# proycon/colibri-core

Measured on AMD Instinct MI355X. Metric: M patterns counted/sec at n<=5 thr=2; identical pattern set vs reference, higher is better.
Workload: dtype u64; 1 GPU; 100000000-token-per-GPU synthetic Zipf(1.0, V=1000000) class-encoded corpus (.colibri.dat v2), sentences 5..35 tokens, unindexed PatternModel<uint32_t>, MAXLENGTH=5, MINTOKENS=2; patterns_in_model=9386566, parallelism=single device

## Files before the change

### colibri-core_amd/csrc/bigram2.hpp

```cpp
#pragma once
#ifndef COLIBRI_BI2_HUGE
#define COLIBRI_BI2_HUGE 16384
#endif
#include "bi2_mix.hpp"
#include "binned.hpp"

namespace colibri {

#ifndef COLIBRI_BI2_CNT16
#define COLIBRI_BI2_CNT16 1
#endif
#ifndef COLIBRI_BI2_WEU
#define COLIBRI_BI2_WEU 4
#endif
constexpr int bi2_count_weu(int slots, bool key4, bool based) { return (COLIBRI_BI2_CNT16 && slots == 1024 && !key4 && !based) ? 5 : COLIBRI_BI2_WEU; }
#ifndef COLIBRI_BI2_WROWS
#define COLIBRI_BI2_WROWS 12
#endif
#ifndef COLIBRI_BI2_WSLOTS
#define COLIBRI_BI2_WSLOTS 1024
#endif
#ifndef COLIBRI_BI2_BINTARGET
#define COLIBRI_BI2_BINTARGET 700
#endif
// ... 1232 lines not shown
        const uint32_t excl = bi2_block_scan<kBi2BigThreads>(nk, &ktotal, wsumL);
        bi2_block_scan<kBi2BigThreads>(nu, &distinct, wsumL);
        if (distinct > kMaxLoad || ktotal > 1023u) {
            if (tid == 0) bs->overflow = 2;
            continue;
        }
        if (tid == 0) {
            atomicAdd(&bs->found_part[a], distinct);
            bs->binkept[a * kBi2BBins + b] = ktotal;
            if (ktotal) atomicAdd(&bs->kept_part[a], ktotal);
        }
        if (ktotal == 0) {
            if (KEY4)
                for (uint32_t j = tid; j < total; j += kBi2BigThreads) code_at[locate(j)] = kInvalid;
            continue;
        }
        const bool reps_lds = ktotal <= (uint32_t)kBi2WReps;
        {
            uint32_t r = excl;
#pragma unroll
            for (uint32_t i = 0; i < per; ++i) {
                if (cS[i] >= threshold) {
                    sp_cnt[spo + r] = cS[i];
                    cntT[s0 + i]    = kBi2Kept | r;
                    if (reps_lds)
                        repS[r] = 0xFFFFFFFFu;
                    else
                        sp_rep[spo + r] = 0xFFFFFFFFu;
                    ++r;
                }
            }
        }
        if (!reps_lds) __threadfence();
        __syncthreads();
        const uint32_t fcode = (a * (uint32_t)kBi2BBins + b) << 10;
        for (uint32_t j0 = 0; j0 < total; j0 += kBi2BigRows * kBi2BigThreads) {
            load4(j0);
#pragma unroll
            for (int q = 0; q < kBi2BigRows; ++q) {
                if (j0 + q * kBi2BigThreads + (tid & ~(uint32_t)(kWave - 1)) >= total) continue;
                const bool     valid = y[q] != ~0ull;
                const uint32_t key = (uint32_t)(y[q] >> pb) & 0x7FFFFFFFu;
                uint32_t       pos = (uint32_t)(y[q] & pmask);
                if (PDROP && pdsh != 0u) {
                    uint32_t jj = j0 + q * kBi2BigThreads + tid, sub = 0;
#pragma unroll
                    for (int s2 = 0; s2 < NSUB - 1; ++s2) {
                        const bool beyond = jj >= rn[s2] && sub == (uint32_t)s2;
                        jj -= beyond ? rn[s2] : 0u;
                        sub += beyond ? 1u : 0u;
                    }
                    const uint32_t sh = pdsh - 1u;
                    pos               = ((pos >> sh) << (sh + 3u)) | (sub << sh) | (pos & ((1u << sh) - 1u));
                }
                uint32_t       c = 0;
                if (valid) c = cntT[bi2_find(keyT, key, bi2_bucket_of(key, lgb, bmask), bmask)];
                const bool     kept = (c & kBi2Kept) != 0;
                const uint32_t r    = c & ~kBi2Kept;
                if (KEY4 && valid) code_at[pos] = kept ? (fcode | r) : kInvalid;
                if (kept) {
                    if (reps_lds) {
                        if (pos < repS[r]) atomicMin(&repS[r], pos);
                    } else if (pos < __hip_atomic_load(&sp_rep[spo + r], __ATOMIC_RELAXED, __HIP_MEMORY_SCOPE_AGENT)) {
                        atomicMin(&sp_rep[spo + r], pos);
                    }
                }
                if (want_positions && !KEY4) {
                    const uint64_t m = __ballot(kept);
                    const uint32_t n = (uint32_t)__popcll(m);
                    if (n && (chunk == kInvalid || cursor + n > csize)) {
                        if (chunk != kInvalid && lane == 0) wcnt[chunk] = cursor;
                        uint32_t cc = 0;
                        if (lane == 0) cc = atomicAdd(&bs->nextchunk, 1u);
                        cc     = (uint32_t)__builtin_amdgcn_readfirstlane((int)cc);
                        chunk  = cc < pn ? pfirst + cc : kInvalid;
                        cursor = 0;
                        if (chunk == kInvalid) lost = true;
                    }
                    if (kept && chunk != kInvalid) {
                        const size_t at = (size_t)chunk * csize + cursor + (uint32_t)__popcll(m & ((1ull << lane) - 1ull));
                        wlist[at]       = pos;
                        if (wcode != nullptr) wcode[at] = fcode | r;
                    }
                    if (chunk != kInvalid) cursor += n;
                }
            }
        }
        __syncthreads();
        if (reps_lds)
            for (uint32_t r = tid; r < ktotal; r += kBi2BigThreads) sp_rep[spo + r] = repS[r];
    }
    if (want_positions && chunk != kInvalid && lane == 0) wcnt[chunk] = cursor;
    if (__any(lost) && lane == 0) bs->overflow = 3;
}

__global__ void bi2_chunk_cursor_kernel(Bi2State* __restrict__ bs, uint32_t* __restrict__ keep, bool restore) {
    if (restore)
        bs->nextchunk = *keep;
    else
        *keep = bs->nextchunk;
}
__global__ __launch_bounds__(kBi2BBins) void bi2_kept_scan_kernel(Bi2State* __restrict__ bs, const DevState* __restrict__ st) {
    if (st->done) return;
    __shared__ uint32_t inL[kBi2BBins], outL[kBi2BBins], wsumL[8], beforeL;
    const uint32_t      a = blockIdx.x;
    inL[threadIdx.x]      = threadIdx.x < a ? bs->kept_part[threadIdx.x] : 0u;
    __syncthreads();
    const uint32_t before = bi2_scan512(inL, outL, wsumL);
    if (threadIdx.x == 0) beforeL = before;
    __syncthreads();
    inL[threadIdx.x] = bs->binkept[a * kBi2BBins + threadIdx.x];
    __syncthreads();
    const uint32_t tot                        = bi2_scan512(inL, outL, wsumL);
    bs->binkept[a * kBi2BBins + threadIdx.x] = beforeL + outL[threadIdx.x];
    if (a == kBins - 1 && threadIdx.x == 0) bs->kept_bins = beforeL + tot;
}
__global__ __launch_bounds__(kBlock) void bi2_finish_kernel(DevState* __restrict__ st, Bi2State* __restrict__ bs, uint32_t threshold, uint32_t res_cap,
                                                             uint32_t* __restrict__ headsurv_keep ,
                                                             uint32_t ovf_code = 4 ) {
    if (st->done) return;
    uint32_t htot, ftot, hftot;
    block_exclusive_scan(bs->found_part[threadIdx.x], &ftot);
    static_assert(kBi2HeadN == kBlock * 16, "16 head keys per lane");
    uint32_t hk = 0, hf = 0, bits = 0;
#pragma unroll
    for (int q = 0; q < 16; ++q) {
        const uint32_t c = bs->headcnt[threadIdx.x * 16 + q];
        hf += c != 0;
        if (c >= threshold) {
            ++hk;
            bits |= 1u << q;
        }
    }
    reinterpret_cast<uint16_t*>(bs->headsurv)[threadIdx.x] = (uint16_t)bits;
    if (headsurv_keep != nullptr) reinterpret_cast<uint16_t*>(headsurv_keep)[threadIdx.x] = (uint16_t)bits;
    const uint32_t ho = block_exclusive_scan(hk, &htot);
    bs->headbase[threadIdx.x] = ho;
    block_exclusive_scan(hf, &hftot);
    if (threadIdx.x == 0) {
        const uint32_t tot = bs->kept_bins;
        bs->kept_head      = htot;
        bs->ran            = 1;
        bs->res_base       = st->res_total + st->kept;
        st->found += ftot + hftot;
        st->kept += tot + htot;
        if ((uint64_t)bs->res_base + tot + htot > res_cap) st->overflow = 1;
        if (bs->overflow && st->radix_overflow != 4) st->radix_overflow = ovf_code;
        const uint64_t next = (uint64_t)st->id_base + bs->nrec;
        if (next >= 0xFFFFFFF0ull) st->radix_overflow = 3;
        st->id_base = (uint32_t)next;
    }
}
__global__ __launch_bounds__(kBi2BBins) void bi2_kept_finish_kernel(DevState* __restrict__ st, Bi2State* __restrict__ bs, uint32_t threshold, uint32_t res_cap,
                                                                     uint32_t* __restrict__ headsurv_keep, uint32_t ovf_code) {
    if (st->done) return;
    __shared__ uint32_t inL[kBi2BBins], outL[kBi2BBins], wsumL[8], beforeL;
    if (blockIdx.x < (uint32_t)kBins) {
        const uint32_t a = blockIdx.x;
        inL[threadIdx.x] = threadIdx.x < a ? bs->kept_part[threadIdx.x] : 0u;
        __syncthreads();
        const uint32_t before = bi2_scan512(inL, outL, wsumL);
        if (threadIdx.x == 0) beforeL = before;
        __syncthreads();
        inL[threadIdx.x] = bs->binkept[a * kBi2BBins + threadIdx.x];
        __syncthreads();
        const uint32_t tot                        = bi2_scan512(inL, outL, wsumL);
        bs->binkept[a * kBi2BBins + threadIdx.x] = beforeL + outL[threadIdx.x];
        if (a == kBins - 1 && threadIdx.x == 0) bs->kept_bins = beforeL + tot;
        return;
    }
    static_assert(kBi2HeadN == kBlock * 16 && kBins == kBlock && kBi2BBins >= kBlock, "16 head keys per lane of the first 256");
    const bool low = threadIdx.x < (uint32_t)kBlock;
    uint32_t   htot, ftot, hftot, tot;
    bi2_block_scan<kBi2BBins>(low ? bs->found_part[threadIdx.x] : 0u, &ftot, wsumL);
    bi2_block_scan<kBi2BBins>(low ? bs->kept_part[threadIdx.x] : 0u, &tot, wsumL);
    uint32_t hk = 0, hf = 0, bits = 0;
    if (low) {
#pragma unroll
        for (int q = 0; q < 16; ++q) {
            const uint32_t c = bs->headcnt[threadIdx.x * 16 + q];
            hf += c != 0;
            if (c >= threshold) {
                ++hk;
                bits |= 1u << q;
            }
        }
        reinterpret_cast<uint16_t*>(bs->headsurv)[threadIdx.x] = (uint16_t)bits;
        if (headsurv_keep != nullptr) reinterpret_cast<uint16_t*>(headsurv_keep)[threadIdx.x] = (uint16_t)bits;
    }
    const uint32_t ho = bi2_block_scan<kBi2BBins>(hk, &htot, wsumL);
    if (low) bs->headbase[threadIdx.x] = ho;
    bi2_block_scan<kBi2BBins>(hf, &hftot, wsumL);
    if (threadIdx.x == 0) {
        bs->kept_head = htot;
        bs->ran       = 1;
        bs->res_base  = st->res_total + st->kept;
        st->found += ftot + hftot;
        st->kept += tot + htot;
        if ((uint64_t)bs->res_base + tot + htot > res_cap) st->overflow = 1;
        if (bs->overflow && st->pad[0] == 0) st->pad[0] = bs->overflow | (bs->kbits << 8) | (bs->posbits << 16) | (bs->bshift << 24);
        if (bs->overflow && st->radix_overflow != 4) st->radix_overflow = ovf_code;
        const uint64_t next = (uint64_t)st->id_base + bs->nrec;
        if (next >= 0xFFFFFFF0ull) st->radix_overflow = 3;
        st->id_base = (uint32_t)next;
    }
}
__global__ __launch_bounds__(kBlock) void bi2_compact_kernel(const uint32_t* __restrict__ sp_rep, const uint32_t* __restrict__ sp_cnt, const DevState* __restrict__ st,
                                                              const Bi2State* __restrict__ bs, uint32_t* __restrict__ res_rep, uint32_t* __restrict__ res_cnt, uint32_t res_cap,
                                                              bool beside = false ) {
    if (beside ? !bs->ran : st->done != 0) return;
    const uint32_t res_base = bs->res_base, lane = threadIdx.x & (kWave - 1);
    if (blockIdx.x + 1 < gridDim.x) {
        const uint32_t nwaves = (gridDim.x - 1) * (kBlock / kWave);
        for (uint32_t g = blockIdx.x * (kBlock / kWave) + threadIdx.x / kWave; g < (uint32_t)kBi2Final; g += nwaves) {
            const uint32_t f   = ((g & (uint32_t)(kBins - 1)) * kBi2BBins) + (g >> 8);
            const uint32_t off = bs->binkept[f];
            const uint32_t n   = ((f + 1 < (uint32_t)kBi2Final) ? bs->binkept[f + 1] : bs->kept_bins) - off;
            if (n == 0) continue;
            const uint32_t src = bs->binoff[f];
            for (uint32_t j = lane; j < n; j += kWave) {
                const uint32_t r = res_base + off + j;
                if (r < res_cap) {
                    res_rep[r] = sp_rep[src + j];
                    res_cnt[r] = sp_cnt[src + j];
                }
            }
        }
    } else {
        uint32_t       r    = res_base + bs->kept_bins + bs->headbase[threadIdx.x];
        const uint32_t bits = reinterpret_cast<const uint16_t*>(bs->headsurv)[threadIdx.x];
#pragma unroll
        for (int q = 0; q < 16; ++q)
            if (bits & (1u << q)) {
                if (r < res_cap) {
                    res_rep[r] = ~bs->headposinv[threadIdx.x * 16 + q];
                    res_cnt[r] = bs->headcnt[threadIdx.x * 16 + q];
                }
                ++r;
            }
    }
}

template <int PER>
struct Bi2PospartLdsT {
    uint32_t stgL[kBi2Threads * PER], stgC[kBi2Threads * PER];
    uint16_t binL[kBi2Threads * PER];
    uint32_t histL[kBi2Buckets], offL[kBi2Buckets], gbaseL[kBi2Buckets], wsumL[kBi2Threads / kWave];
};
using Bi2PospartLds = Bi2PospartLdsT<kBi2Per>;
#ifndef COLIBRI_PP_PER
#define COLIBRI_PP_PER 4
#endif
constexpr int kBi2PpPer = COLIBRI_PP_PER;
template <int PER>
__device__ __forceinline__ void bi2_pospart_tile(Bi2PospartLdsT<PER>& L, const uint32_t (&p)[PER], const uint32_t (&code)[PER], uint32_t shard, Bi2State* __restrict__ bs,
                                                 DevState* __restrict__ st, uint32_t* __restrict__ plist, Bi2Lists pl, uint32_t* __restrict__ pcode) {
    static_assert(kBi2Buckets == kBi2Threads, "one lane per position bucket");
    uint32_t rank[PER];
    KP_INIT(3);
    L.histL[threadIdx.x] = 0;
    __syncthreads();
    KP(0);
#pragma unroll
    for (int k = 0; k < PER; ++k) {
        rank[k] = kInvalid;
        if (p[k] != 0xFFFFFFFFu) {
            const uint32_t b = p[k] >> pl.pshift;
            rank[k]          = atomicAdd(&L.histL[b], 1u) | (b << 16);
        }
    }
    __syncthreads();
    KP(1);
    uint32_t tot;
    L.offL[threadIdx.x] = bi2_block_scan<kBi2Threads>(L.histL[threadIdx.x], &tot, L.wsumL);
    __syncthreads();
    KP(2);
    const uint32_t rs_h = L.histL[threadIdx.x], rs_l = shard * kBi2Buckets + threadIdx.x;
    uint32_t       rs_at = 0;
    if (rs_h) rs_at = atomicAdd(&bs->pcur[bi2_pc(rs_l)], rs_h);
#pragma unroll
    for (int k = 0; k < PER; ++k) {
        if (rank[k] != kInvalid) {
            const uint32_t b = rank[k] >> 16, q = L.offL[b] + (rank[k] & 0xFFFFu);
            L.stgL[q]        = p[k];
            L.stgC[q]        = code[k];
            L.binL[q]        = (uint16_t)b;
        }
    }
    {
        uint32_t g = 0;
        if (rs_h) {
            if (rs_at + rs_h > pl.pcap) st->radix_overflow = 4;
            g = rs_l * pl.pcap + min(rs_at, pl.pcap - min(pl.pcap, rs_h));
        }
        L.gbaseL[threadIdx.x] = g;
    }
    __syncthreads();
    KP(3);
    for (uint32_t j = threadIdx.x; j < tot; j += kBi2Threads) {
        const uint32_t b                           = L.binL[j];
        plist[(size_t)L.gbaseL[b] + (j - L.offL[b])] = L.stgL[j];
        if (pcode != nullptr) pcode[(size_t)L.gbaseL[b] + (j - L.offL[b])] = L.stgC[j];
    }
    __syncthreads();
    KP(4);
    KP_DONE();
}
__global__ __launch_bounds__(kBi2Threads, kBi2PpPer <= 4 ? kBi2Threads / 128 : 4) void bi2_pospart_kernel(const uint32_t* __restrict__ wlist, const uint32_t* __restrict__ wcnt, uint32_t nlists, uint32_t wcap,
                                                                                      Bi2State* __restrict__ bs, DevState* __restrict__ st, uint32_t* __restrict__ plist, Bi2Lists pl,
                                                                                      const uint32_t* __restrict__ wcode = nullptr, uint32_t* __restrict__ pcode = nullptr,
                                                                                      uint32_t flat_n = 0, bool dense = false) {
    if (st->done) return;
    __shared__ Bi2PospartLdsT<kBi2PpPer> L;
    const uint32_t           shard = blockIdx.x & (uint32_t)(kBi2Shards - 1);
    auto                     tile  = [&](uint32_t (&p)[kBi2PpPer], uint32_t (&code)[kBi2PpPer]) {
        if (dense) {
#pragma unroll
            for (int k = 0; k < kBi2PpPer; ++k)
                if (p[k] != 0xFFFFFFFFu) code[k] = bs->binkept[code[k] >> 10] + (code[k] & 1023u);
        }
        bi2_pospart_tile(L, p, code, shard, bs, st, plist, pl, pcode);
    };
    if (flat_n) {
        for (uint32_t w = blockIdx.x; w < nlists; w += gridDim.x) {
            const uint32_t        n    = min(wcap, flat_n - min(flat_n, w * wcap));
            const uint32_t* const src  = wlist + (size_t)w * wcap;
            const uint32_t* const csrc = wcode != nullptr ? wcode + (size_t)w * wcap : nullptr;
            for (uint32_t j0 = 0; j0 < n; j0 += kBi2Threads * kBi2PpPer) {
                uint32_t p[kBi2PpPer], code[kBi2PpPer];
#pragma unroll
                for (int k = 0; k < kBi2PpPer; ++k) {
                    const uint32_t j = j0 + k * kBi2Threads + threadIdx.x;
                    p[k]             = j < n ? src[j] : 0xFFFFFFFFu;
                    code[k]          = (csrc != nullptr && j < n) ? csrc[j] : 0u;
                }
                tile(p, code);
            }
        }
        return;
    }
    __shared__ uint32_t cntL[kBi2Threads];
    static_assert(2 * (sizeof(Bi2PospartLdsT<kBi2PpPer>) + sizeof(uint32_t) * kBi2Threads) <= 160 * 1024, "two blocks per CU (the launches' 512 blocks on 256 CUs) share its 160 KB of LDS");
    const uint32_t      mine = blockIdx.x < nlists ? (nlists - blockIdx.x + gridDim.x - 1) / gridDim.x : 0u;
    for (uint32_t i0 = 0; i0 < mine; i0 += kBi2Threads) {
        const uint32_t ni = min((uint32_t)kBi2Threads, mine - i0);
        if (threadIdx.x < ni) cntL[threadIdx.x] = min(wcnt[blockIdx.x + (i0 + threadIdx.x) * gridDim.x], wcap);
        __syncthreads();
        auto     len = [&](uint32_t i_) { return i_ < ni ? (uint32_t)__builtin_amdgcn_readfirstlane((int)cntL[i_]) : 0u; };
        uint32_t i = 0, off = 0, ci = len(0);
        for (;;) {
            uint32_t p[kBi2PpPer], code[kBi2PpPer];
            bool     any = false;
#pragma unroll
            for (int k = 0; k < kBi2PpPer; ++k) {
                while (i < ni && off >= ci) {
                    ++i;
                    off = 0;
                    ci  = len(i);
                }
                p[k]    = 0xFFFFFFFFu;
                code[k] = 0u;
                if (i < ni) {
                    any              = true;
                    const uint32_t j = off + threadIdx.x;
                    if (j < ci) {
// ... 141 lines not shown
```

### colibri-core_amd/csrc/chain.hpp

```cpp
#pragma once
#include "bigram2.hpp"
#include "chain_step.hpp"

namespace colibri {

#ifndef COLIBRI_CH_THREADS
#define COLIBRI_CH_THREADS 512
#endif
constexpr int kChThreads = COLIBRI_CH_THREADS;
constexpr int kChPer     = 4;
constexpr int kChStep    = kChThreads * kChPer;
constexpr int kChQueue   = 2 * kChStep;
constexpr int kChQueueLds = kChQueue - kChThreads;
constexpr uint32_t kChSliceShift = 17;
constexpr uint32_t kChSliceWords = ((1u << kChSliceShift) / 32u + 1u + 3u) & ~3u;
#ifndef COLIBRI_CH_RUN
#define COLIBRI_CH_RUN 2
#endif
constexpr uint32_t kChRun = COLIBRI_CH_RUN;
constexpr int kChEmitBlocks = 3;
constexpr size_t kLdsPerCu = 160 * 1024;

#ifndef COLIBRI_CH_HUGE
#define COLIBRI_CH_HUGE 4096
// ... 132 lines not shown
        const uint32_t per = (nwords + kBi2BmThreads - 1) / kBi2BmThreads, w0 = threadIdx.x * per, w1 = min(nwords, w0 + per);
        uint32_t       mine = 0;
        for (uint32_t w = w0; w < w1; ++w) mine += (uint32_t)__popc(bmL[w]);
        uint32_t total;
        uint32_t run = bi2_block_scan<kBi2BmThreads>(mine, &total, redL);
        for (uint32_t w = w0; w < w1; ++w) {
            wpre[(start >> 5) + w] = run;
            run += (uint32_t)__popc(bmL[w]);
        }
        if (threadIdx.x == 0) btot[b] = total;
    }
    for (int off = 32; off > 0; off >>= 1) nset += __shfl_down(nset, off, kWave);
    if ((threadIdx.x & (kWave - 1)) == 0) redL[threadIdx.x / kWave] = nset;
    __syncthreads();
    if (threadIdx.x == 0) {
        uint32_t v = 0;
        for (int w = 0; w < kBi2BmThreads / kWave; ++w) v += redL[w];
        if (v) atomicAdd(&st->valid, v);
    }
}

template <int QCAP>
struct ChainQueueT {
    static constexpr int kQPer = QCAP / kChThreads;
    static_assert(QCAP % kChThreads == 0 && QCAP > kChStep, "flush: kQPer entries per lane; a step's candidates fit behind what waits");
    unsigned long long* qL;
    uint8_t*            qaL;
    uint32_t *          histL, *offL, *gbaseL, *wsumL;
    uint32_t            qn;
    uint32_t            nadm;
    __device__ __forceinline__ void flush(unsigned long long* __restrict__ recsA, uint32_t region, uint32_t sub, Bi2State* __restrict__ bs) {
        __syncthreads();
        if (threadIdx.x < kBins) histL[threadIdx.x] = 0;
        __syncthreads();
        unsigned long long r[kQPer];
        uint32_t           rk[kQPer];
#pragma unroll
        for (int q = 0; q < kQPer; ++q) {
            const uint32_t j = q * kChThreads + threadIdx.x;
            r[q]             = 0;
            rk[q]            = kInvalid;
            if (j < qn) {
                r[q]             = qL[j];
                const uint32_t a = qaL[j];
                rk[q]            = atomicAdd(&histL[a], 1u) | (a << 16);
            }
        }
        __syncthreads();
        bi2_scan256(histL, offL, wsumL);
        uint32_t rs_at = 0, rs_h = 0;
        if (threadIdx.x < kBins) {
            rs_h = histL[threadIdx.x];
            if (rs_h) rs_at = atomicAdd(&bs->curA[bi2_cur(sub * kBins + threadIdx.x)], rs_h);
        }
#pragma unroll
        for (int q = 0; q < kQPer; ++q) {
            if (rk[q] != kInvalid) {
                const uint32_t a = rk[q] >> 16, p = offL[a] + (rk[q] & 0xFFFFu);
                qL[p]            = r[q];
                qaL[p]           = (uint8_t)a;
            }
        }
        if (threadIdx.x < kBins) {
            uint32_t g = 0;
            if (rs_h) {
                const uint32_t slot = sub * kBins + threadIdx.x;
                if (rs_at + rs_h > region) bs->overflow = 1;
                g = slot * region + min(rs_at, region - min(region, rs_h));
            }
            gbaseL[threadIdx.x] = g;
        }
        __syncthreads();
        for (uint32_t j = threadIdx.x; j < qn; j += kChThreads) {
            const uint32_t a                         = qaL[j];
            recsA[(size_t)gbaseL[a] + (j - offL[a])] = qL[j];
        }
        __syncthreads();
        qn = 0;
    }
};
static_assert(kChStep / kChThreads == kChPer && kChThreads >= kBins && kChThreads % kWave == 0 && kChThreads / kWave <= 16, "bi2_scan256 / bi2_block_scan");

struct ChainKey {
    uint32_t           K, clsbits, pb;
    uint32_t           pshift, pdrop;
    unsigned long long kmask;
    template <class Queue>
    __device__ __forceinline__ void put(Queue& q, uint32_t at, uint32_t dn, uint32_t cn, uint32_t pos) const {
        const uint64_t m = bi2_mix(((uint64_t)dn << clsbits) | cn, K);
        if (pdrop) pos = ((pos >> (pshift + 3)) << pshift) | (pos & ((1u << pshift) - 1u));
        q.qL[at]  = ((m & kmask) << pb) | pos;
        q.qaL[at] = (uint8_t)(m >> (K - 8));
    }
};
__device__ __forceinline__ bool chain_key_bits(const Bi2State* __restrict__ prev, uint32_t clsbits, uint32_t pb, Bi2State* __restrict__ bs, ChainKey& ck, uint32_t hugebin = 0,
                                               uint32_t kfix = 0, uint32_t pshift = 0, uint32_t pdrop = 0) {
    const uint32_t kept_prev = prev->kept_bins + prev->kept_head;
    uint32_t       idbits    = 1;
    while (idbits < 32 && (1ull << idbits) < (uint64_t)kept_prev + 1) ++idbits;
    const uint32_t K = kfix ? kfix : max(idbits + clsbits, 17u);
    if (threadIdx.x == 0) {
        bs->kbits   = K;
        bs->posbits = pb;
        bs->hugebin = hugebin ? hugebin : kChHugeBin;
        bs->pdshift = pdrop ? pshift + 1u : 0u;
    }
    ck.pshift = pshift;
    ck.pdrop  = pdrop;
    if ((!kfix && K > 48u) || K - 8u + pb > 64u) {
        if (threadIdx.x == 0) bs->overflow = 1;
        return false;
    }
    ck.K       = K;
    ck.clsbits = clsbits;
    ck.pb      = pb;
    ck.kmask   = (1ull << (K - 8)) - 1ull;
    return true;
}

#define CHAIN_QUEUE_LDS_N(q, QCAP)                                                               \
    __shared__ unsigned long long q##_qL[QCAP];                                                  \
    __shared__ uint8_t            q##_qaL[QCAP];                                                 \
    __shared__ uint32_t           q##_histL[kBins], q##_offL[kBins], q##_gbaseL[kBins], q##_wsumL[kChThreads / kWave]; \
    ChainQueueT<QCAP> q{q##_qL, q##_qaL, q##_histL, q##_offL, q##_gbaseL, q##_wsumL, 0u, 0u}
#define CHAIN_QUEUE_LDS(q) CHAIN_QUEUE_LDS_N(q, kChQueue)
constexpr size_t chain_queue_lds_bytes(int qcap) { return (size_t)qcap * 9 + 3 * kBins * 4 + (kChThreads / kWave) * 4; }

constexpr uint32_t kChXcds = 8;
__device__ __forceinline__ void chain_number_steps(const Bi2State* __restrict__ prev, const Bi2Lists& pl, uint32_t nbuckets, uint2* __restrict__ table, uint32_t cap,
                                                   uint32_t* __restrict__ nsteps, uint32_t x, uint32_t* wsumL) {
    constexpr uint32_t kPer = (kBi2Buckets / kChXcds * kChLists + kBi2Threads - 1) / kBi2Threads;
    uint32_t           first[kPer], n[kPer], ns[kPer], bucket[kPer], sum = 0;
#pragma unroll
    for (uint32_t q = 0; q < kPer; ++q) {
        const uint32_t idx = threadIdx.x * kPer + q, bkt = x + kChXcds * (idx / kChLists), shard = idx % kChLists;
        uint32_t       lcap = 0;
        first[q] = n[q] = 0;
        bucket[q]       = bkt;
        if (bkt < nbuckets) {
            bi2_list_of(pl, shard, bkt, first[q], lcap);
            n[q] = min(prev->pcur[bi2_pc(shard * kBi2Buckets + bkt)], lcap);
        }
        ns[q] = (n[q] + kChStep - 1) / kChStep;
        sum += ns[q];
    }
    uint32_t total;
    uint32_t base = bi2_block_scan<kBi2Threads>(sum, &total, wsumL);
#pragma unroll
    for (uint32_t q = 0; q < kPer; ++q)
        for (uint32_t k = 0; k < ns[q]; ++k, ++base)
            if (base < cap) table[(size_t)x * cap + base] = make_uint2(first[q] + k * (uint32_t)kChStep, chain_step_pack(min((uint32_t)kChStep, n[q] - k * (uint32_t)kChStep), bucket[q]));
    if (threadIdx.x == 0) nsteps[x] = min(total, cap);
}
__global__ __launch_bounds__(kBi2Threads) void chain_steps_kernel(const Bi2State* __restrict__ prev, Bi2Lists pl, uint32_t nbuckets, uint2* __restrict__ table, uint32_t cap,
                                                                   uint32_t* __restrict__ nsteps, const DevState* __restrict__ st) {
    if (st->done) return;
    __shared__ uint32_t wsumL[kBi2Threads / kWave];
    chain_number_steps(prev, pl, nbuckets, table, cap, nsteps, blockIdx.x, wsumL);
}
constexpr uint32_t kChResetBlocks = 64;
__global__ __launch_bounds__(kBi2Threads) void chain_begin_kernel(const Bi2State* __restrict__ prev, Bi2Lists pl, uint32_t nbuckets, uint2* __restrict__ table, uint32_t cap,
                                                                   uint32_t* __restrict__ nsteps, const DevState* __restrict__ st, Bi2State* __restrict__ bs, uint32_t* __restrict__ wcnt,
                                                                   uint32_t nwcnt) {
    if (blockIdx.x >= kChXcds) {
        chain_clear_state(bs, wcnt, nwcnt, (blockIdx.x - kChXcds) * kBi2Threads + threadIdx.x, (gridDim.x - kChXcds) * kBi2Threads);
        return;
    }
    if (st->done) return;
    __shared__ uint32_t wsumL[kBi2Threads / kWave];
    chain_number_steps(prev, pl, nbuckets, table, cap, nsteps, blockIdx.x, wsumL);
}
inline uint32_t chain_steps_cap(const Bi2Lists& pl) { return (kBi2Buckets / kChXcds) * (kBi2Shards * (pl.pcap / kChStep + 1) + ((1u << pl.pshift) / kChStep + 1)); }

template <bool BITS_LDS>
__global__ __launch_bounds__(kChThreads, kChEmitBlocks* kChThreads / 256) void chain_emit_kernel(
    const uint32_t* __restrict__ cls, uint32_t npos, uint32_t n, uint32_t clsbits, uint32_t pb, const Bi2State* __restrict__ prev, const uint32_t* __restrict__ plist,
    const uint32_t* __restrict__ pcode, Bi2Lists pl, const uint2* __restrict__ table, uint32_t cap, const uint32_t* __restrict__ nsteps, const uint32_t* __restrict__ bitmap,
    unsigned long long* __restrict__ recsA, uint32_t region, uint32_t nsub, Bi2State* __restrict__ bs, DevState* __restrict__ st, const uint32_t* __restrict__ headid ,
    uint32_t dbg = 0, uint32_t kfix = 0, uint32_t pdrop = 0 ) {
    if (st->done) return;
    ChainKey ck;
    if (!chain_key_bits(prev, clsbits, pb, bs, ck, dbg >> 8, kfix, pl.pshift, pdrop)) return;
    constexpr int      kQCap = BITS_LDS ? kChQueueLds : kChQueue;
    constexpr uint32_t kRun = BITS_LDS ? kChRun : 1u, kSliceL = BITS_LDS ? kChSliceWords : 4u;
    CHAIN_QUEUE_LDS_N(Q, kQCap);
    __shared__ __attribute__((aligned(16))) uint32_t sliceL[kSliceL];
    static_assert(kChEmitBlocks * ((chain_queue_lds_bytes(kQCap) + kSliceL * 4 + 2047) / 2048 * 2048) <= kLdsPerCu, "kChEmitBlocks blocks of chain_emit_kernel per CU");
    const uint32_t        sub = blockIdx.x % nsub;
    const uint32_t        x = blockIdx.x % kChXcds, nper = gridDim.x / kChXcds, ns = nsteps[x];
    const uint2* const    tab = table + (size_t)x * cap;
    const uint32_t        rbase = kfix ? 0u : prev->res_base;
    uint32_t              k = chain_run_first(blockIdx.x / kChXcds, kRun), k1 = chain_run_next(k, nper, kRun);
    constexpr uint32_t kSlicePer = BITS_LDS ? ((1u << kChSliceShift) / 128u + kChThreads - 1) / kChThreads : 1u;
    const uint32_t     sw = (1u << pl.pshift) / 32u + 1u, tw = (npos + 31u) / 32u + 16u;
    uint32_t           stail = 0, snw = 0;
    auto               slice_fetch = [&](uint32_t bucket) {
        const uint32_t w0 = bucket << (pl.pshift - 5u);
        snw               = min(sw, tw - w0);
#pragma unroll
        for (uint32_t u = 0; u < kSlicePer; ++u) {
            const uint32_t g0 = u * kChThreads + (threadIdx.x & ~(uint32_t)(kWave - 1)), g = u * kChThreads + threadIdx.x;
            if (g < (snw >> 2)) {
                uint32_t off = 16u * g;
                asm volatile("" : "+v"(off));
                __builtin_amdgcn_global_load_lds((const __attribute__((address_space(1))) void*)(reinterpret_cast<const char*>(bitmap + w0) + off),
                                                 (__attribute__((address_space(3))) void*)(sliceL + 4u * g0), 16, 0, 0);
            }
        }
        if (threadIdx.x < (snw & 3u)) stail = bitmap[w0 + (snw & ~3u) + threadIdx.x];
    };
    auto slice_store = [&]() {
        if (threadIdx.x < (snw & 3u)) sliceL[(snw & ~3u) + threadIdx.x] = stail;
        asm volatile("s_waitcnt vmcnt(0)" ::: "memory");
    };
    uint32_t ps[kChPer], code[kChPer];
    bool     ok[kChPer];
    auto     entry = [&](uint32_t s) -> uint2 {
        const uint2 e = s < ns ? tab[s] : make_uint2(0u, 0u);
        return make_uint2((uint32_t)__builtin_amdgcn_readfirstlane((int)e.x), (uint32_t)__builtin_amdgcn_readfirstlane((int)e.y));
    };
    uint2 e1 = entry(k);
    auto  load_pairs = [&]() {
        const uint32_t np = chain_step_pairs(e1.y);
#pragma unroll
        for (int q = 0; q < kChPer; ++q) {
            const uint32_t j = q * kChThreads + threadIdx.x;
            ok[q]            = j < np;
            ps[q]            = ok[q] ? plist[(size_t)e1.x + j] : 0u;
            code[q]          = ok[q] ? pcode[(size_t)e1.x + j] : 0u;
        }
    };
    load_pairs();
    uint32_t bcur = chain_step_bucket(e1.y);
    if (BITS_LDS && k < ns) {
        slice_fetch(bcur);
        slice_store();
        __syncthreads();
    }
    e1 = entry(k1);
    KP_INIT(4);
    while (k < ns) {
        uint32_t p2[kChPer], c2[kChPer], w[kChPer], cn[kChPer];
        bool     k2[kChPer];
#pragma unroll
        for (int q = 0; q < kChPer; ++q) {
            p2[q] = ps[q];
            c2[q] = code[q];
            k2[q] = ok[q];
        }
        const uint32_t start = bcur << pl.pshift;
#pragma unroll
        for (int q = 0; q < kChPer; ++q) {
            if (BITS_LDS)
                w[q] = (k2[q] && !(dbg & 1u)) ? sliceL[(p2[q] + 1u - start) >> 5] : 0x55555555u;
            else
                w[q] = (k2[q] && !(dbg & 1u)) ? bitmap[(p2[q] + 1u) >> 5] : 0x55555555u;
        }
        load_pairs();
        bool reload = false;
        if (BITS_LDS && k1 < ns && chain_step_bucket(e1.y) != bcur) {
            reload = true;
            bcur   = chain_step_bucket(e1.y);
        }
        k  = k1;
        k1 = chain_run_next(k1, nper, kRun);
        e1 = entry(k1);
        uint32_t cnt = 0;
#pragma unroll
        for (int q = 0; q < kChPer; ++q) {
            k2[q] = k2[q] && ((w[q] >> ((p2[q] + 1u) & 31u)) & 1u);
            if (k2[q] && (c2[q] & kBi2HeadCode)) {
                const uint32_t r = headid[c2[q] & 0xFFFu];
                k2[q]            = r != kInvalid;
                c2[q]            = r - rbase;
            }
            cnt += k2[q] ? 1u : 0u;
        }
        KP(0);
#pragma unroll
        for (int q = 0; q < kChPer; ++q)
            cn[q] = (k2[q] && !(dbg & 2u)) ? cls[p2[q] + n - 1u] : (p2[q] & 1023u);
        uint32_t total;
        uint32_t at = Q.qn + bi2_block_scan<kChThreads>(cnt, &total, Q.wsumL);
        KP(1);
        if (reload) slice_fetch(bcur);
#pragma unroll
        for (int q = 0; q < kChPer; ++q)
            if (k2[q]) ck.put(Q, at++, c2[q] , cn[q], p2[q]);
        Q.qn += total;
        Q.nadm += total;
        KP(2);
        if (reload) {
            slice_store();
            __syncthreads();
        }
        if (Q.qn >= (uint32_t)(kQCap - kChStep)) {
            Q.flush(recsA, region, sub, bs);
            KP(3);
        }
    }
    KP_DONE();
    if (Q.qn) Q.flush(recsA, region, sub, bs);
    if (threadIdx.x == 0 && Q.nadm) atomicAdd(&st->admitted, Q.nadm);
    bi2_offsets_tail(bs, region, nsub, Q.histL, Q.offL, Q.wsumL, Q.gbaseL);
}

template <bool HEAD>
__global__ __launch_bounds__(kChThreads, 6) void skip_emit_kernel(const uint32_t* __restrict__ list, const uint32_t* __restrict__ nlist, const uint32_t* __restrict__ left, uint32_t offl,
                                                                   const uint32_t* __restrict__ right, uint32_t offr, uint32_t l_is_cls, uint32_t r_is_cls, uint32_t clsbits, uint32_t pb,
                                                                   unsigned long long* __restrict__ recsA, uint32_t region, uint32_t nsub, Bi2State* __restrict__ bs, DevState* __restrict__ st,
                                                                   uint32_t* __restrict__ head_rows = nullptr) {
    if (st->done) return;
    __shared__ uint32_t headL[HEAD ? kBi2HeadN : 1], hposL[HEAD ? kBi2HeadN : 1];
    if (HEAD) {
        for (int k = threadIdx.x; k < kBi2HeadN; k += kChThreads) {
            headL[k] = 0;
            hposL[k] = 0xFFFFFFFFu;
        }
        __syncthreads();
    }
    auto flush_head = [&]() {
        if (HEAD) {
            __syncthreads();
            uint32_t* const row = head_rows + (size_t)blockIdx.x * (2 * kBi2HeadN);
            for (int k = threadIdx.x; k < kBi2HeadN; k += kChThreads) {
                row[k]             = headL[k];
                row[kBi2HeadN + k] = hposL[k];
            }
        }
    };
    uint32_t idb = 1;
    while (idb < 32 && (1ull << idb) < (uint64_t)st->res_total + 1) ++idb;
    const uint32_t lbits = l_is_cls ? clsbits : idb, rbits = r_is_cls ? clsbits : idb;
    ChainKey       ck;
    if (lbits + rbits > 48u) {
        if (threadIdx.x == 0) bs->overflow = 1;
        flush_head();
        return;
    }
    if (!chain_key_bits(bs, rbits, pb, bs, ck, 0, max(lbits + rbits, 17u))) {
        flush_head();
        return;
    }
    CHAIN_QUEUE_LDS(Q);
    const uint32_t sub = blockIdx.x % nsub, n = *nlist;
    for (uint32_t t0 = blockIdx.x * (uint32_t)kChStep; t0 < n; t0 += gridDim.x * (uint32_t)kChStep) {
        uint32_t p[kChPer], l[kChPer], r[kChPer], cnt = 0;
        bool     ok[kChPer];
#pragma unroll
        for (int q = 0; q < kChPer; ++q) {
            const uint32_t j = t0 + q * kChThreads + threadIdx.x;
            ok[q]            = j < n;
            p[q]             = ok[q] ? list[j] : 0u;
        }
#pragma unroll
        for (int q = 0; q < kChPer; ++q) {
            l[q] = ok[q] ? left[p[q] + offl] : 0u;
            r[q] = ok[q] ? right[p[q] + offr] : 0u;
        }
#pragma unroll
        for (int q = 0; q < kChPer; ++q) {
            ok[q] = ok[q] && l[q] != kInvalid && r[q] != kInvalid;
            if (HEAD && ok[q] && l[q] < (uint32_t)kBi2Head && r[q] < (uint32_t)kBi2Head) {
                const uint32_t h = l[q] * kBi2Head + r[q];
                atomicAdd(&headL[h], 1u);
                atomicMin(&hposL[h], p[q]);
                ok[q] = false;
            }
            cnt += ok[q] ? 1u : 0u;
        }
        uint32_t total;
        uint32_t at = Q.qn + bi2_block_scan<kChThreads>(cnt, &total, Q.wsumL);
#pragma unroll
        for (int q = 0; q < kChPer; ++q)
            if (ok[q]) ck.put(Q, at++, l[q], r[q], p[q]);
        Q.qn += total;
        Q.nadm += total;
        if (Q.qn >= (uint32_t)kChStep) Q.flush(recsA, region, sub, bs);
    }
    if (Q.qn) Q.flush(recsA, region, sub, bs);
    flush_head();
    if (threadIdx.x == 0 && Q.nadm) atomicAdd(&st->admitted, Q.nadm);
    bi2_offsets_tail(bs, region, nsub, Q.histL, Q.offL, Q.wsumL, Q.gbaseL);
}

__global__ __launch_bounds__(kChThreads) void chain_ids_kernel(const uint32_t* __restrict__ plist, const uint32_t* __restrict__ pcode, const uint2* __restrict__ table, uint32_t cap,
                                                                const uint32_t* __restrict__ nsteps, const Bi2State* __restrict__ bs, const DevState* __restrict__ st,
                                                                uint32_t* __restrict__ ids, const uint32_t* __restrict__ headid = nullptr ) {
    if (st->done) return;
    const uint32_t     x = blockIdx.x % kChXcds, nper = gridDim.x / kChXcds, ns = nsteps[x], res_base = bs->res_base;
    const uint2* const tab = table + (size_t)x * cap;
    for (uint32_t k = blockIdx.x / kChXcds; k < ns; k += nper) {
        const uint2    e  = tab[k];
        const uint32_t np = chain_step_pairs(e.y);
        uint32_t       ps[kChPer], cd[kChPer];
#pragma unroll
        for (int q = 0; q < kChPer; ++q) {
            const uint32_t j = q * kChThreads + threadIdx.x;
            ps[q]            = j < np ? plist[(size_t)e.x + j] : kInvalid;
            cd[q]            = j < np ? pcode[(size_t)e.x + j] : 0u;
        }
#pragma unroll
        for (int q = 0; q < kChPer; ++q)
            if (ps[q] != kInvalid) ids[ps[q]] = (headid != nullptr && (cd[q] & kBi2HeadCode)) ? headid[cd[q] & 0xFFFu] : res_base + cd[q];
    }
}

struct ChainPairsOut {
    const uint32_t*           wpre;
    const uint32_t*           btot;
    const uint4*              blocks;
    const unsigned long long* chain;
    unsigned long long*       pairs;
    uint32_t*                 pay;
    unsigned long long        pcap;
    int                       which;
    uint32_t                  sb, tb;
};
__global__ __launch_bounds__(kBi2Threads) void chain_ids_full_kernel(const uint32_t* __restrict__ plist, const uint32_t* __restrict__ pcode, Bi2Lists pl, uint32_t nbuckets, uint32_t plog,
                                                                      uint32_t npos, const Bi2State* __restrict__ bs, const DevState* __restrict__ st, uint32_t* __restrict__ ids ,
                                                                      const uint32_t* __restrict__ headid, ChainPairsOut po) {
    if (st->done) return;
    extern __shared__ uint32_t idsL[];
    __shared__ uint32_t        wsumL[kBi2Threads / kWave];
    const uint32_t xcd = blockIdx.x % kChXcds, part = (blockIdx.x / kChXcds) & ((1u << plog) - 1u), bucket = (blockIdx.x / (kChXcds << plog)) * kChXcds + xcd;
    if (bucket >= nbuckets) return;
    const uint32_t wlen = (1u << pl.pshift) >> plog, start = (bucket << pl.pshift) + part * wlen;
    if (start >= npos) return;
    for (uint32_t k = threadIdx.x; k < wlen; k += kBi2Threads) idsL[k] = kInvalid;
    __syncthreads();
    const uint32_t res_base = bs->res_base, nl = headid != nullptr ? kChLists : (uint32_t)kBi2Shards;
    uint32_t first[kChLists], nn[kChLists], nmax = 0;
#pragma unroll
    for (uint32_t x = 0; x < kChLists; ++x) {
        uint32_t cap = 0;
        first[x] = nn[x] = 0;
        if (x < nl) {
            bi2_list_of(pl, x, bucket, first[x], cap);
            nn[x] = min(bs->pcur[bi2_pc(x * kBi2Buckets + bucket)], cap);
        }
        nmax = max(nmax, nn[x]);
    }
    auto put = [&](uint32_t pos, uint32_t at) {
        const uint32_t o = pos - start;
        if (o < wlen) {
            const uint32_t cd = pcode[at];
            idsL[o]           = (headid != nullptr && (cd & kBi2HeadCode)) ? headid[cd & 0xFFFu] : res_base + cd;
        }
    };
    for (uint32_t j = threadIdx.x; j * 4u < nmax; j += kBi2Threads) {
        uint4 e[kChLists];
#pragma unroll
        for (uint32_t x = 0; x < kChLists; ++x)
            e[x] = j * 4u < nn[x] ? reinterpret_cast<const uint4*>(plist + first[x])[j] : make_uint4(0u, 0u, 0u, 0u);
#pragma unroll
        for (uint32_t x = 0; x < kChLists; ++x) {
            const uint32_t at = first[x] + 4u * j, left = nn[x] > 4u * j ? nn[x] - 4u * j : 0u;
            if (left > 0u) put(e[x].x, at);
            if (left > 1u) put(e[x].y, at + 1u);
            if (left > 2u) put(e[x].z, at + 2u);
            if (left > 3u) put(e[x].w, at + 3u);
        }
    }
    __syncthreads();
    const uint32_t m = min(wlen, npos - start);
    if (ids != nullptr)
        for (uint32_t k = threadIdx.x; k < m; k += kBi2Threads) ids[start + k] = idsL[k];
    if (po.wpre == nullptr) return;
    uint32_t before = 0;
    for (uint32_t k = threadIdx.x; k < bucket; k += kBi2Threads) before += po.btot[k];
    uint32_t btotal;
    bi2_block_scan<kBi2Threads>(before, &btotal, wsumL);
    constexpr uint32_t kW   = kBi2Threads / kWave;
    const uint32_t     lane = threadIdx.x & (kWave - 1), wave = threadIdx.x / kWave;
    const uint32_t     rows = (m + kWave - 1) / kWave, rper = (rows + kW - 1) / kW, r0 = wave * rper, r1 = min(rows, r0 + rper);
    uint32_t           mine = 0;
    for (uint32_t r = r0; r < r1; ++r) {
        const uint32_t k = r * kWave + lane;
        mine += (uint32_t)__popcll(__ballot(k < m && idsL[k] != kInvalid));
    }
    uint32_t       ptotal;
    const uint32_t wexcl = bi2_block_scan<kBi2Threads>(lane == 0 ? mine : 0u, &ptotal, wsumL);
    const uint32_t wbase = (uint32_t)__shfl((int)wexcl, 0, kWave);
    const uint32_t tmask = po.tb >= 32 ? 0xFFFFFFFFu : (1u << po.tb) - 1u;
    uint64_t       o     = po.chain[po.which] + btotal + po.wpre[start >> 5] + wbase;
    for (uint32_t r = r0; r < r1; ++r) {
        const uint32_t k = r * kWave + lane, p = start + k;
        const uint32_t id = k < m ? idsL[k] : kInvalid;
        const uint64_t mk = __ballot(id != kInvalid);
        if (mk == 0) continue;
        const uint4 rb = po.blocks[p >> 6];
        if (id != kInvalid) {
            const uint64_t at = o + (uint32_t)__popcll(mk & ((1ull << lane) - 1ull));
            if (at < po.pcap) {
                const uint32_t bit   = p & 63u;
                const uint64_t below = ((((uint64_t)rb.w << 32) | rb.z)) & ((1ull << bit) - 1ull);
                const uint32_t sent = rb.x + (uint32_t)__popcll(below), tok = below ? bit - (64u - (uint32_t)__clzll(below)) : p - rb.y;
                if (po.pay != nullptr) {
                    reinterpret_cast<uint32_t*>(po.pairs)[at] = id;
                    po.pay[at]                                = (sent << po.tb) | (tok & tmask);
                } else {
                    po.pairs[at] = ((unsigned long long)id << (po.sb + po.tb)) | ((unsigned long long)sent << po.tb) | (tok & tmask);
                }
            }
        }
        o += (uint32_t)__popcll(mk);
    }
}

__global__ __launch_bounds__(kChThreads) void chain_pairs_kernel(const uint32_t* __restrict__ plist, const uint32_t* __restrict__ pcode, const uint2* __restrict__ table, uint32_t cap,
                                                                  const uint32_t* __restrict__ nsteps, const Bi2State* __restrict__ bs, const DevState* __restrict__ st,
                                                                  const uint32_t* __restrict__ bitmap, const uint32_t* __restrict__ wpre, const uint32_t* __restrict__ btot,
                                                                  uint32_t nbuckets, uint32_t pshift, const uint4* __restrict__ blocks, const unsigned long long* __restrict__ chain,
                                                                  int which, uint64_t pcap, unsigned long long* __restrict__ pairs, uint32_t* __restrict__ pay, uint32_t sb, uint32_t tb,
                                                                  const uint32_t* __restrict__ headid) {
    if (st->done) return;
    __shared__ uint32_t bbaseL[kBi2Buckets], wsumL[kChThreads / kWave];
    static_assert(kBi2Buckets == 2 * kChThreads, "two buckets per lane");
    {
        const uint32_t b0 = 2 * threadIdx.x, t0 = b0 < nbuckets ? btot[b0] : 0u, t1 = b0 + 1 < nbuckets ? btot[b0 + 1] : 0u;
        uint32_t       total;
        const uint32_t excl = bi2_block_scan<kChThreads>(t0 + t1, &total, wsumL);
        bbaseL[b0]     = excl;
        bbaseL[b0 + 1] = excl + t0;
    }
    __syncthreads();
    const uint32_t     x = blockIdx.x % kChXcds, nper = gridDim.x / kChXcds, ns = nsteps[x], res_base = bs->res_base;
    const uint2* const tab   = table + (size_t)x * cap;
    const uint64_t     obase = chain[which];
    const uint32_t     tmask = tb >= 32 ? 0xFFFFFFFFu : (1u << tb) - 1u;
    for (uint32_t k = blockIdx.x / kChXcds; k < ns; k += nper) {
        const uint2    e  = tab[k];
        const uint32_t np = chain_step_pairs(e.y);
        uint32_t       ps[kChPer], cd[kChPer], bw[kChPer], wp[kChPer];
        uint4          r[kChPer];
#pragma unroll
        for (int q = 0; q < kChPer; ++q) {
            const uint32_t j = q * kChThreads + threadIdx.x;
            ps[q]            = j < np ? plist[(size_t)e.x + j] : kInvalid;
            cd[q]            = j < np ? pcode[(size_t)e.x + j] : 0u;
        }
#pragma unroll
        for (int q = 0; q < kChPer; ++q) {
            const uint32_t p = ps[q] != kInvalid ? ps[q] : 0u;
            bw[q]            = bitmap[p >> 5];
            wp[q]            = wpre[p >> 5];
            r[q]             = blocks[p >> 6];
        }
#pragma unroll
        for (int q = 0; q < kChPer; ++q) {
            if (ps[q] == kInvalid) continue;
            const uint32_t p = ps[q];
            if (!((bw[q] >> (p & 31u)) & 1u)) continue;
            const uint32_t id  = (headid != nullptr && (cd[q] & kBi2HeadCode)) ? headid[cd[q] & 0xFFFu] : res_base + cd[q];
            const uint64_t o   = obase + bbaseL[p >> pshift] + wp[q] + (uint32_t)__popc(bw[q] & ((1u << (p & 31u)) - 1u));
            if (o >= pcap) continue;
            const uint32_t bit = p & 63u;
            const uint64_t below = ((((uint64_t)r[q].w << 32) | r[q].z)) & ((1ull << bit) - 1ull);
            const uint32_t sent = r[q].x + (uint32_t)__popcll(below), tok = below ? bit - (64u - (uint32_t)__clzll(below)) : p - r[q].y;
            if (pay != nullptr) {
                reinterpret_cast<uint32_t*>(pairs)[o] = id;
                pay[o]                                = (sent << tb) | (tok & tmask);
            } else
                pairs[o] = ((unsigned long long)id << (sb + tb)) | ((unsigned long long)sent << tb) | (tok & tmask);
        }
    }
}

__global__ __launch_bounds__(kBlock) void chain_alist_kernel(const uint32_t* __restrict__ bitmap, uint32_t npos, const DevState* __restrict__ st, uint32_t* __restrict__ list_out,
                                                              uint32_t* __restrict__ nlist_out) {
    if (st->done) return;
    __shared__ uint32_t baseL, wsumL[kBlock / kWave];
    constexpr uint32_t  kPerLane = 8;
    const uint32_t      nwords = (npos + 31) / 32, ntiles = (nwords + kBlock * kPerLane - 1) / (kBlock * kPerLane);
    for (uint32_t tile = blockIdx.x; tile < ntiles; tile += gridDim.x) {
        const uint32_t w0 = (tile * kBlock + threadIdx.x) * kPerLane;
        uint32_t       y[kPerLane], cnt = 0;
        uint32_t       x = w0 < nwords ? bitmap[w0] : 0u;
#pragma unroll
        for (uint32_t k = 0; k < kPerLane; ++k) {
            const uint32_t nx = w0 + k + 1 <= nwords ? bitmap[w0 + k + 1] : 0u;
            y[k]              = w0 + k < nwords ? x & ((x >> 1) | (nx << 31)) : 0u;
            cnt += (uint32_t)__popc(y[k]);
            x = nx;
        }
        uint32_t       total;
        const uint32_t excl = bi2_block_scan<kBlock>(cnt, &total, wsumL);
        if (threadIdx.x == 0) baseL = total ? atomicAdd(nlist_out, total) : 0u;
        __syncthreads();
        uint32_t o = baseL + excl;
#pragma unroll
        for (uint32_t k = 0; k < kPerLane; ++k) {
            uint32_t yy = y[k];
            while (yy) {
                list_out[o++] = (w0 + k) * 32 + (uint32_t)__builtin_ctz(yy);
                yy &= yy - 1;
            }
        }
        __syncthreads();
    }
}

}
```

### colibri-core_amd/csrc/chain_step.hpp

```cpp
#pragma once
#include <stdint.h>

#if defined(__HIPCC__) || defined(__CUDACC__)
#define COLIBRI_STEP_HD __host__ __device__ __forceinline__
#else
#define COLIBRI_STEP_HD inline
#endif

namespace colibri {

constexpr uint32_t kChStepPairBits = 16;
COLIBRI_STEP_HD uint32_t chain_step_pack(uint32_t pairs, uint32_t bucket) { return pairs | (bucket << kChStepPairBits); }
COLIBRI_STEP_HD uint32_t chain_step_pairs(uint32_t y) { return y & ((1u << kChStepPairBits) - 1u); }
COLIBRI_STEP_HD uint32_t chain_step_bucket(uint32_t y) { return y >> kChStepPairBits; }

COLIBRI_STEP_HD uint32_t chain_run_first(uint32_t k, uint32_t run) { return k * run; }
COLIBRI_STEP_HD uint32_t chain_run_next(uint32_t s, uint32_t nper, uint32_t run) { return (s + 1u) % run != 0u ? s + 1u : s + 1u + (nper - 1u) * run; }

}
```

### colibri-core_amd/csrc/colibri_hip.hip

```cpp
#include <hip/hip_runtime.h>

#include <algorithm>
#include <chrono>
#include <cstdarg>
#include <cstdio>
#include <cstring>
#include <functional>
#include <new>
#include <string>
#include <utility>
#include <vector>

#include "colibri_hip.h"
#include "binned.hpp"
#include "bigram2.hpp"
#include "chain.hpp"
#include "kshard.hpp"
#include "kshard2.hpp"
#include "textenc.hpp"
#include "constrained.hpp"
#include "flexgrams.hpp"
#include "cooc.hpp"
#include "relations.hpp"
#include "skiprel.hpp"
// ... 875 lines not shown
        hipLaunchKernelGGL(bin_offsets_kernel, dim3(1), dim3(kBlock), 0, c->stream, c->binstate.p, region);
        hipLaunchKernelGGL(bin_hist2_kernel, dim3(tiles + kBins), dim3(kBlock), 0, c->stream, c->recs[0].p, c->state.p, c->binstate.p);
        hipLaunchKernelGGL(bin_scan2_kernel, dim3(kBins), dim3(kBlock), 0, c->stream, c->binstate.p);
        hipLaunchKernelGGL(bin_scatter_kernel, dim3(tiles + kBins), dim3(kBlock), 0, c->stream, c->recs[0].p, c->recs[1].p, c->state.p, c->binstate.p);
    }
    const BinnedIO io = binned_planes(c, pl, with_keys);
    {
        static const int walk_mode = getenv("COLIBRI_BIN_WALK") ? atoi(getenv("COLIBRI_BIN_WALK")) : 0;
        if (walk_mode) HIP_TRY(c, hipMemcpyAsync(&c->binstate.p->walk_mode, &walk_mode, sizeof(uint32_t), hipMemcpyHostToDevice, c->stream));
        Prof p(c, COLIBRI_K_BINCOUNT);
        hipLaunchKernelGGL(bin_count_kernel, dim3(256 * 12), dim3(kBlock), 0, c->stream, c->recs[1].p, c->state.p, c->binstate.p, thr, io.sp_rep, io.sp_cnt, io.sp_key, ids_at, flags_at, dense_code);
    }
    return COLIBRI_OK;
}

int binned_resolve_stage(colibri_ctx* c, const TrainPlan& pl, uint32_t* ids_out, int n, bool use_list, bool build_list, const uint32_t* remap, uint32_t remap_base,
                         bool prefill_ids = true, bool decode = false, uint32_t decode_base = 0, const uint32_t* list_other = nullptr, const uint32_t* nlist_other = nullptr) {
    const uint32_t* list_in   = list_other ? list_other : c->alist[n & 1].p;
    const uint32_t* nlist_in  = list_other ? nlist_other : c->alist_n.p + (n & 1);
    uint32_t*       list_out  = build_list ? c->alist[(n + 1) & 1].p : nullptr;
    uint32_t*       nlist_out = c->alist_n.p + ((n + 1) & 1);
    if (build_list || !list_other) HIP_TRY(c, hipMemsetAsync(nlist_out, 0, sizeof(uint32_t), c->stream));
    if (use_list && prefill_ids) HIP_TRY(c, hipMemsetAsync(ids_out, 0xFF, sizeof(uint32_t) * (size_t)pl.npos, c->stream));
    Prof p(c, COLIBRI_K_RESOLVE);
    if (use_list)
        hipLaunchKernelGGL((bin_resolve_kernel<true>), dim3(pl.pos_grid), dim3(kBlock), 0, c->stream, c->rep_of.p, c->ids_at.p, ids_out, c->state.p, pl.npos, list_in, nlist_in, list_out,
                           nlist_out, remap, remap_base, decode ? (const BinState*)c->binstate.p : (const BinState*)nullptr, decode_base);
    else
        hipLaunchKernelGGL((bin_resolve_kernel<false>), dim3(pl.pos_grid), dim3(kBlock), 0, c->stream, c->rep_of.p, c->ids_at.p, ids_out, c->state.p, pl.npos, (const uint32_t*)nullptr,
                           (const uint32_t*)nullptr, list_out, nlist_out, remap, remap_base, decode ? (const BinState*)c->binstate.p : (const BinState*)nullptr, decode_base);
    return COLIBRI_OK;
}

#ifndef COLIBRI_BI2_WPC
#define COLIBRI_BI2_WPC 20
#endif
#ifndef COLIBRI_BI2_SUB
#define COLIBRI_BI2_SUB 4
#endif
constexpr uint32_t kBi2Sub = COLIBRI_BI2_SUB, kBi2SubWide = 8, kBi2EmitGrid = 512, kBi2Waves = 256 * COLIBRI_BI2_WPC;
thread_local bool tl_small_passes = false;
inline uint64_t slice_env() {
    static const uint64_t env = [] {
        const char* e = getenv("COLIBRI_SLICE_POSITIONS");
        return (uint64_t)(e ? strtoull(e, nullptr, 10) : 0ull);
    }();
    return env;
}
inline uint64_t slice_positions() { return slice_env() ? std::min<uint64_t>(slice_env(), 110ull * 1000 * 1000) : 110ull * 1000 * 1000; }
constexpr uint64_t kNarrowPassPositions = 215ull * 1000 * 1000, kWidePassPositions = 430ull * 1000 * 1000;
inline uint64_t single_pass_positions() { return slice_env() ? slice_env() : tl_small_passes ? 110ull * 1000 * 1000 : kWidePassPositions; }
inline bool retry_with_small_passes(uint64_t npos) { return !tl_small_passes && !slice_env() && npos > 110ull * 1000 * 1000; }
inline uint64_t big_corpus_tokens() { return slice_env() ? slice_env() : tl_small_passes ? 128ull * 1000 * 1000 : 400ull * 1000 * 1000; }
inline bool chain_fits(uint64_t npos) { return slice_env() ? true : npos <= kNarrowPassPositions; }
inline bool chain_wide(uint64_t npos) {
    static const bool force = getenv("COLIBRI_FORCE_WIDE_CHAIN") != nullptr;
    return force || (!slice_env() && npos > kNarrowPassPositions);
}
inline bool chain_fits_plain(uint64_t npos) { return chain_fits(npos) || (npos <= kWidePassPositions && !getenv("COLIBRI_NO_WIDE_CHAIN")); }
constexpr uint32_t kBi2TailPerWave = 2;
inline uint32_t bi2_tail() {
    const char* e = getenv("COLIBRI_BI2_TAIL");
    return e && *e ? (uint32_t)std::min(1l << 20, std::max(0l, atol(e))) : kBi2TailPerWave * (uint32_t)(kBi2Waves / kBi2Shards);
}
inline uint32_t slice_bits(uint64_t records) {
    if (records <= single_pass_positions()) return 0;
    uint32_t s = 1;
    while (s < 6 && ((slice_positions() * 14 / 11) << s) < records) ++s;
    return s;
}
struct Bigram2Plan {
    uint32_t nslots, region, pshift, nbuckets, wcap, wextra, clsbits, posbits, sbits;
    size_t   listn;
    Bi2Lists pl;
};
Bigram2Plan bigram2_plan(const colibri_ctx* c, uint32_t npos, uint32_t nsub = kBi2Sub) {
    Bigram2Plan b{};
    b.nslots = kBins * nsub;
    b.region = (uint32_t)(std::min<uint64_t>(2ull * c->recs[0].n, 2ull * c->recs[1].n) / b.nslots);
    if (slice_bits(npos)) b.region = (uint32_t)std::min<uint64_t>(b.region, (slice_positions() * 5 / 2) / b.nslots + 8192);
    b.pshift = 12;
    while (((uint64_t)npos >> b.pshift) > (uint64_t)kBi2Buckets - 1) ++b.pshift;
    b.nbuckets  = std::max<uint32_t>(1u, (uint32_t)(((uint64_t)npos + (1u << b.pshift) - 1) >> b.pshift));
    b.pl.pshift = b.pshift;
    b.pl.pcap   = ((1u << b.pshift) / 4 + 4096 + 3) & ~3u;
    b.pl.hbase  = kBi2Shards * kBi2Buckets * b.pl.pcap;
    b.listn     = (size_t)b.pl.hbase + ((size_t)b.nbuckets << b.pshift) + 64;
    const uint32_t resident = (!slice_env() && npos > kNarrowPassPositions) ? std::min(kBi2Waves, 256u * 9u) : kBi2Waves;
    b.wcap      = (uint32_t)(((uint64_t)npos * 6 / 10 / resident) * 2 + 4096);
    b.wextra    = npos / b.wcap + kBi2Waves + 64;
    b.clsbits   = 1;
    while ((1ull << b.clsbits) <= (uint64_t)c->maxclass) ++b.clsbits;
    b.posbits = 1;
    while ((1ull << b.posbits) < (uint64_t)npos + 1) ++b.posbits;
    b.posbits = std::max(b.posbits, 27u);
    b.sbits   = slice_bits(npos);
    return b;
}
bool bigram2_fits(const colibri_ctx* c, uint32_t npos) {
    const Bigram2Plan b = bigram2_plan(c, npos);
    return npos < (1u << kBi2MaxPosBits) && 2 * b.clsbits - b.sbits - 8 + b.posbits <= 64;
}
inline bool bi2_keep_enabled() {
    const char* const e = getenv("COLIBRI_BI2_KEEP");
    return !(e && e[0] == '0' && e[1] == 0);
}
void bi2_keep_alloc(colibri_ctx* c, const Bigram2Plan& b) {
    auto& k = c->b2.keep;
    if (b.sbits != 0 || c->ks.active || c->sh.active || !bi2_keep_enabled()) return;
    const size_t nrec = (size_t)b.nslots * b.region, nboff = (size_t)kBins * kBi2SubWide * (kBi2BBins + 1);
    if (k.recs.p && k.recs.n >= nrec && k.boff.p && k.boff.n >= nboff && k.snap.p) return;
    if (k.refused && nrec >= k.refused) return;
    k.drop();
    auto reserve = [&](auto& buf, size_t n) {
        using T = std::remove_reference_t<decltype(*buf.p)>;
        if (buf.p && buf.n >= n) return true;
        buf.reset();
        if (hipMalloc(reinterpret_cast<void**>(&buf.p), n * sizeof(T)) != hipSuccess) {
            buf.p = nullptr;
            (void)hipGetLastError();
            return false;
        }
        buf.n = n;
        return true;
    };
    if (reserve(k.recs, nrec) && reserve(k.boff, nboff) && reserve(k.snap, 1) &&
        hipMemsetAsync(k.snap.p, 0, sizeof(Bi2Keep), c->stream) == hipSuccess)
        return;
    (void)hipGetLastError();
    k.refused = nrec;
    k.recs.reset();
    k.boff.reset();
    k.snap.reset();
}
inline bool bi2_keep_room(const colibri_ctx* c, const Bigram2Plan& b) {
    const auto& k = c->b2.keep;
    return k.recs.p && k.recs.n >= (size_t)b.nslots * b.region && k.boff.p && k.snap.p;
}
int bigram2_alloc(colibri_ctx* c, uint32_t npos, bool chain = false, bool keep = false ) {
    const Bigram2Plan b = bigram2_plan(c, npos);
    int               rc;
    if ((rc = dev_alloc(c, c->b2.state, 1)) || (rc = dev_alloc(c, c->b2.boff, (size_t)kBins * kBi2SubWide * (kBi2BBins + 1))) ||
        (rc = dev_alloc(c, c->b2.head_rows, (size_t)kBi2EmitGrid * 2 * kBi2HeadN)) || (rc = dev_alloc(c, c->b2.wlist, (size_t)(kBi2Waves + b.wextra) * b.wcap)) ||
        (rc = dev_alloc(c, c->b2.wcnt, (size_t)kBi2Waves + b.wextra + 1)) || (rc = dev_alloc(c, c->b2.plist, chain ? b.listn : (size_t)kBi2Shards * kBi2Buckets * b.pl.pcap + 64)) ||
        (rc = dev_alloc(c, c->b2.bitmap, (size_t)npos / 32 + 24)) || (rc = dev_alloc(c, c->b2.headsurv, kBi2HeadN / 32)))
        return rc;
    if (chain && c->b2.aux == nullptr) {
        HIP_TRY(c, hipStreamCreateWithFlags(&c->b2.aux, hipStreamNonBlocking));
        HIP_TRY(c, hipEventCreateWithFlags(&c->b2.ev_fork, hipEventDisableTiming));
        HIP_TRY(c, hipEventCreateWithFlags(&c->b2.ev_join, hipEventDisableTiming));
        HIP_TRY(c, hipEventCreateWithFlags(&c->b2.ev_fork2, hipEventDisableTiming));
        HIP_TRY(c, hipEventCreateWithFlags(&c->b2.ev_join2, hipEventDisableTiming));
    }
    if (chain && ((rc = dev_alloc(c, c->b2.steps, 2 * (size_t)kChXcds * chain_steps_cap(b.pl) + kChXcds)) || (rc = dev_alloc(c, c->b2.state2, 1)) || (rc = dev_alloc(c, c->b2.state3, 1)) || (rc = dev_alloc(c, c->b2.wcode, (size_t)(kBi2Waves + b.wextra) * b.wcap)) ||
                  (rc = dev_alloc(c, c->b2.pcode, b.listn)) || (rc = dev_alloc(c, c->b2.headid, kBi2HeadN))))
        return rc;
    if (b.sbits) {
        if ((rc = dev_alloc(c, c->b2.sid, (size_t)npos + 64))) return rc;
        HIP_TRY(c, hipMemsetAsync(c->b2.sid.p + (npos & ~15u), 0xFF, 64, c->stream));
    }
    if (keep) bi2_keep_alloc(c, b);
    if (!c->b2.attr_set) {
        HIP_TRY(c, hipFuncSetAttribute((const void*)bi2_bitmap_kernel, hipFuncAttributeMaxDynamicSharedMemorySize, (int)(((size_t)1 << kBi2MaxPosBits) / kBi2Buckets / 8)));
        HIP_TRY(c, hipFuncSetAttribute((const void*)chain_bitmap_kernel, hipFuncAttributeMaxDynamicSharedMemorySize, (int)(((size_t)1 << kBi2MaxPosBits) / kBi2Buckets / 8)));
        c->b2.attr_set = true;
    }
    return COLIBRI_OK;
}
int chain_compact_fork(colibri_ctx* c, const BinnedIO& io, const Bi2State* bs, const TrainPlan& pl) {
    HIP_TRY(c, hipEventRecord(c->b2.ev_fork2, c->stream));
    HIP_TRY(c, hipStreamWaitEvent(c->b2.aux, c->b2.ev_fork2, 0));
    hipLaunchKernelGGL(bi2_compact_kernel, dim3(1025), dim3(kBlock), 0, c->b2.aux, (const uint32_t*)io.sp_rep, (const uint32_t*)io.sp_cnt, (const DevState*)c->state.p, bs, c->res_rep.p,
                       c->res_cnt.p, pl.res_cap, true);
    HIP_TRY(c, hipEventRecord(c->b2.ev_join2, c->b2.aux));
    c->b2.compact_pending = true;
    return COLIBRI_OK;
}
int chain_compact_join(colibri_ctx* c) {
    if (!c->b2.compact_pending) return COLIBRI_OK;
    HIP_TRY(c, hipStreamWaitEvent(c->stream, c->b2.ev_join2, 0));
    c->b2.compact_pending = false;
    return COLIBRI_OK;
}
inline uint32_t chain_grid(const char* env_name, uint32_t dflt) {
    const char* e = getenv(env_name);
    const long  v = e ? atol(e) : 0;
    if (v <= 0 || v > 65536) return dflt;
    return (uint32_t)((v + 7) / 8 * 8);
}
static_assert(8 % COLIBRI_BI2_SUB == 0, "chain_grid rounds to multiples of 8");
inline uint32_t chain_dbg() {
#ifdef COLIBRI_DEBUG_KNOBS
    static const uint32_t v = getenv("COLIBRI_CH_DBG") ? (uint32_t)atoi(getenv("COLIBRI_CH_DBG")) : 0u;
    return v;
#else
    return 0u;
#endif
}
inline bool chain_bits_lds(const Bi2Lists& pl) {
    const char* const e = getenv("COLIBRI_CH_BITS_LDS");
    return pl.pshift <= kChSliceShift && !(e && e[0] == '0' && e[1] == 0);
}
inline bool chain_ids_full_applies(const Bigram2Plan& b) {
    static const bool scatter = getenv("COLIBRI_IDS_SCATTER") != nullptr;
    return !scatter && b.pshift <= 18;
}
int chain_ids(colibri_ctx* c, const Bigram2Plan& b, const Bi2State* bs, uint32_t* ids, const uint32_t* headid, bool pairs = false) {
    if (chain_ids_full_applies(b)) {
        ChainPairsOut po{};
        if (pairs) {
            po.wpre   = c->b2.wpre.p;
            po.btot   = c->b2.btot.p;
            po.blocks = reinterpret_cast<const uint4*>(c->pos_blocks.p);
            po.chain  = c->pair_chain.p;
            po.pairs  = c->pairs[0].p;
            po.pcap   = c->pairs[0].n;
            po.pay    = c->pair_split ? reinterpret_cast<uint32_t*>(c->pairs[0].p) + po.pcap : (uint32_t*)nullptr;
            po.which  = c->pair_pass;
            po.sb     = c->pair_sb;
            po.tb     = c->pair_tb;
        }
        static const uint32_t plog_min = getenv("COLIBRI_IDS_PLOG") ? (uint32_t)atoi(getenv("COLIBRI_IDS_PLOG")) : 2u;
        const uint32_t plog = std::min(b.pshift, std::max(std::min(plog_min, 6u), b.pshift > 15 ? b.pshift - 15 : 0u));
        if (!c->b2.ids_attr_set) {
            HIP_TRY(c, hipFuncSetAttribute((const void*)chain_ids_full_kernel, hipFuncAttributeMaxDynamicSharedMemorySize, 128 * 1024));
            c->b2.ids_attr_set = true;
        }
        hipLaunchKernelGGL(chain_ids_full_kernel, dim3(((b.nbuckets + kChXcds - 1) / kChXcds) * (kChXcds << plog)), dim3(kBi2Threads), sizeof(uint32_t) << (b.pshift - plog), c->stream,
                           (const uint32_t*)c->b2.plist.p, (const uint32_t*)c->b2.pcode.p, b.pl, b.nbuckets, plog, c->npos, bs, (const DevState*)c->state.p, ids, headid, po);
        if (pairs) {
            hipLaunchKernelGGL(pairs_advance_kernel, dim3(1), dim3(1), 0, c->stream, c->pair_chain.p, c->pair_pass, (const uint32_t*)&c->state.p->valid, po.pcap);
            c->pair_pass ^= 1;
        }
        return COLIBRI_OK;
    }
    if (pairs || ids == nullptr) return fail(c, COLIBRI_ERR_STATE, "chain_ids: pairs need the LDS form");
    HIP_TRY(c, hipMemsetAsync(ids, 0xFF, sizeof(uint32_t) * (size_t)c->npos, c->stream));
    const uint32_t cap = chain_steps_cap(b.pl);
    hipLaunchKernelGGL(chain_steps_kernel, dim3(kChXcds), dim3(kBi2Threads), 0, c->stream, bs, b.pl, b.nbuckets, reinterpret_cast<uint2*>(c->b2.steps.p), cap,
                       c->b2.steps.p + 2 * (size_t)kChXcds * cap, (const DevState*)c->state.p);
    static const uint32_t ids_grid = chain_grid("COLIBRI_IDS_GRID", 1024u);
    hipLaunchKernelGGL(chain_ids_kernel, dim3(ids_grid), dim3(kChThreads), 0, c->stream, (const uint32_t*)c->b2.plist.p, (const uint32_t*)c->b2.pcode.p,
                       reinterpret_cast<const uint2*>(c->b2.steps.p), cap, (const uint32_t*)(c->b2.steps.p + 2 * (size_t)kChXcds * cap), bs, (const DevState*)c->state.p, ids, headid);
    return COLIBRI_OK;
}
void chain_pairs(colibri_ctx* c, const Bigram2Plan& b, const Bi2State* bs, const uint32_t* headid) {
    Prof           p(c, COLIBRI_K_INDEX);
    const uint32_t cap  = chain_steps_cap(b.pl);
    const uint64_t pcap = c->pairs[0].n;
    hipLaunchKernelGGL(chain_steps_kernel, dim3(kChXcds), dim3(kBi2Threads), 0, c->stream, bs, b.pl, b.nbuckets, reinterpret_cast<uint2*>(c->b2.steps.p), cap,
                       c->b2.steps.p + 2 * (size_t)kChXcds * cap, (const DevState*)c->state.p);
    static const uint32_t grid = chain_grid("COLIBRI_IDS_GRID", 1024u);
    hipLaunchKernelGGL(chain_pairs_kernel, dim3(grid), dim3(kChThreads), 0, c->stream, (const uint32_t*)c->b2.plist.p, (const uint32_t*)c->b2.pcode.p,
                       reinterpret_cast<const uint2*>(c->b2.steps.p), cap, (const uint32_t*)(c->b2.steps.p + 2 * (size_t)kChXcds * cap), bs, (const DevState*)c->state.p,
                       (const uint32_t*)c->b2.bitmap.p, (const uint32_t*)c->b2.wpre.p, (const uint32_t*)c->b2.btot.p, b.nbuckets, b.pshift,
                       reinterpret_cast<const uint4*>(c->pos_blocks.p), (const unsigned long long*)c->pair_chain.p, c->pair_pass, pcap, c->pairs[0].p,
                       c->pair_split ? reinterpret_cast<uint32_t*>(c->pairs[0].p) + pcap : (uint32_t*)nullptr, c->pair_sb, c->pair_tb, headid);
    hipLaunchKernelGGL(pairs_advance_kernel, dim3(1), dim3(1), 0, c->stream, c->pair_chain.p, c->pair_pass, (const uint32_t*)&c->state.p->valid, pcap);
    c->pair_pass ^= 1;
}
int bigram2_order(colibri_ctx* c, const TrainPlan& pl, bool want_list, uint32_t* ids_out = nullptr, bool chain = false) {
    const uint32_t    npos = pl.npos, nsurv = c->maxclass / 32 + 1;
    const Bigram2Plan b    = bigram2_plan(c, npos);
    if (ids_out != nullptr) {
        int rc;
        if (b.sbits != 0 || !want_list) return fail(c, COLIBRI_ERR_STATE, "bigram2_order: ids need the single-pass form with lists");
        if ((rc = dev_alloc(c, c->b2.wcode, (size_t)(kBi2Waves + b.wextra) * b.wcap)) || (rc = dev_alloc(c, c->b2.pcode, (size_t)kBi2Shards * kBi2Buckets * b.pl.pcap + 64)) ||
            (rc = dev_alloc(c, c->b2.headid, kBi2HeadN)) || (rc = dev_alloc(c, c->b2.steps, 2 * (size_t)kChXcds * chain_steps_cap(b.pl) + kChXcds)))
            return rc;
    }
    if (chain && b.sbits != 0) return fail(c, COLIBRI_ERR_STATE, "bigram2_order: the chained orders need the single-pass form");
    const bool        with_codes = ids_out != nullptr || (chain && want_list);
    Bi2State* const   bs   = c->b2.state.p;
    auto* const       recsA = reinterpret_cast<unsigned long long*>(c->recs[0].p);
    auto&      kp       = c->b2.keep;
    const bool keepable = b.sbits == 0 && c->b2.surv_known && !c->ks.active && !c->sh.active && bi2_keep_enabled() && bi2_keep_room(c, b);
    uint64_t   key[colibri_ctx::Bigram2::Keep::kKeyWords] = {
        1u, npos, c->maxclass, c->b2.surv_args[0], c->b2.surv_args[1], c->b2.surv_args[2], b.nslots, b.region, b.pshift, b.nbuckets, b.wcap, b.wextra, b.clsbits, b.posbits, b.sbits,
        (uint64_t)b.listn, ((uint64_t)b.pl.pcap << 32) | b.pl.pshift, b.pl.hbase, (chain && want_list) ? 1u : 0u, getenv("COLIBRI_SLICED_EMIT_OFF") ? 1u : 0u};
    const bool reuse = keepable && kp.valid && !kp.pending && std::equal(key, key + colibri_ctx::Bigram2::Keep::kKeyWords, kp.key);
    if (!reuse) {
        kp.drop();
        if (keepable) std::copy(key, key + colibri_ctx::Bigram2::Keep::kKeyWords, kp.key);
    }
    auto* const       recsB = keepable ? kp.recs.p : reinterpret_cast<unsigned long long*>(c->recs[1].p);
    uint32_t* const   boffB = keepable ? kp.boff.p : c->b2.boff.p;
    uint32_t* const   nlist = c->alist_n.p + 1;
    const bool one_reset = chain && b.sbits == 0;
    if (one_reset) {
        if (!reuse) hipLaunchKernelGGL(chain_reset_kernel, dim3(256), dim3(kBlock), 0, c->stream, bs, c->b2.wcnt.p, kBi2Waves + b.wextra + 1);
    } else {
        HIP_TRY(c, hipMemsetAsync(nlist, 0, sizeof(uint32_t), c->stream));
        HIP_TRY(c, hipMemsetAsync(c->b2.wcnt.p, 0, sizeof(uint32_t) * ((size_t)kBi2Waves + b.wextra + 1), c->stream));
    }
    uint32_t* const   keep = c->b2.wcnt.p + kBi2Waves + b.wextra;
    const BinnedIO io = binned_planes(c, pl, false);
    for (uint32_t slice = 0; slice < (1u << b.sbits); ++slice) {
        if (!one_reset && !reuse) HIP_TRY(c, hipMemsetAsync(bs, 0, sizeof(Bi2State), c->stream));
        if (!reuse) {
            Prof p(c, COLIBRI_K_EMIT2);
            if (slice == 0 || b.sbits < 2 || getenv("COLIBRI_SLICED_EMIT_OFF"))
                hipLaunchKernelGGL(bi2_emit_kernel, dim3(kBi2EmitGrid), dim3(kBi2Threads), 0, c->stream, c->cls.p, c->uni_surv.p, nsurv, npos, b.clsbits, b.sbits, slice, b.posbits, recsA,
                                   b.region, kBi2Sub, bs, c->state.p, c->b2.head_rows.p, b.sbits ? c->b2.sid.p : (uint8_t*)nullptr, 0u, (chain && want_list) ? c->b2.plist.p : (uint32_t*)nullptr,
                                   (chain && want_list) ? c->b2.pcode.p : (uint32_t*)nullptr, b.pl);
            else
                hipLaunchKernelGGL(bi2_emit_sliced_kernel, dim3(kBi2EmitGrid), dim3(kBi2Threads), 0, c->stream, c->cls.p, (const uint8_t*)c->b2.sid.p, npos, b.clsbits, b.sbits, slice, b.posbits,
                                   std::max(1u, std::min(8u, 1u << b.sbits) / 4u), recsA, b.region, kBi2Sub, bs, c->state.p);
            if (slice == 0)
                hipLaunchKernelGGL(bi2_head_reduce_kernel, dim3(kBi2HeadN / kBlock, kBi2HeadSplit), dim3(kBlock), 0, c->stream, c->b2.head_rows.p, kBi2EmitGrid, bs, c->state.p);
        }
        if (!reuse) {
            Prof p(c, COLIBRI_K_LEVELB2);
            hipLaunchKernelGGL(bi2_levelB_kernel<false>, dim3(b.nslots), dim3(kBi2Threads), 0, c->stream, recsA, recsB, b.region, bs, boffB, c->state.p);
            hipLaunchKernelGGL(bi2_binoff_kernel, dim3(kBins), dim3(kBi2BBins), 0, c->stream, bs, (const uint32_t*)boffB, kBi2Sub, c->state.p);
            if (keepable) {
                hipLaunchKernelGGL(bi2_keep_kernel, dim3(256), dim3(kBlock), 0, c->stream, bs, kp.snap.p, c->state.p, false, (uint32_t*)nullptr, 0u);
                kp.pending = hipPeekAtLastError() == hipSuccess;
            }
        }
        {
            Prof p(c, COLIBRI_K_COUNT2);
            if (reuse)
                hipLaunchKernelGGL(bi2_keep_kernel, dim3(256), dim3(kBlock), 0, c->stream, bs, kp.snap.p, c->state.p, true, c->b2.wcnt.p, one_reset ? kBi2Waves + b.wextra + 1 : 0u);
            if (b.sbits) hipLaunchKernelGGL(bi2_chunk_cursor_kernel, dim3(1), dim3(1), 0, c->stream, bs, keep, true);
            const bool wide = b.sbits == 0 && !slice_env() && npos > kNarrowPassPositions;
            if (wide)
                hipLaunchKernelGGL((bi2_count_big_kernel<(int)kBi2Sub, false, false, 2048>), dim3(kBi2Waves * kWave / kBi2BigThreads), dim3(kBi2BigThreads), 0, c->stream, recsB, b.region,
                                   (const uint32_t*)boffB, bs, c->state.p, pl.thr, io.sp_rep, io.sp_cnt, c->b2.wlist.p, c->b2.wcnt.p, b.wcap, want_list, with_codes ? c->b2.wcode.p : (uint32_t*)nullptr,
                                   (const uint32_t*)nullptr, kBi2Waves, b.wextra);
            else
            hipLaunchKernelGGL((bi2_count_big_kernel<(int)kBi2Sub>), dim3(kBi2Waves * kWave / kBi2BigThreads), dim3(kBi2BigThreads), 0, c->stream, recsB, b.region, (const uint32_t*)boffB, bs, c->state.p,
                               pl.thr, io.sp_rep, io.sp_cnt, c->b2.wlist.p, c->b2.wcnt.p, b.wcap, want_list, with_codes ? c->b2.wcode.p : (uint32_t*)nullptr, (const uint32_t*)nullptr,
                               kBi2Waves, b.wextra);
            if (b.sbits) hipLaunchKernelGGL(bi2_chunk_cursor_kernel, dim3(1), dim3(1), 0, c->stream, bs, keep, false);
            if (wide)
                hipLaunchKernelGGL((bi2_count_kernel<(int)kBi2Sub, false, kBi2WRows, false, 2048>), dim3(kBi2Waves), dim3(kWave), 0, c->stream, recsB, b.region, (const uint32_t*)boffB, bs, c->state.p,
                                   pl.thr, io.sp_rep, io.sp_cnt, c->b2.wlist.p, c->b2.wcnt.p, b.wcap, want_list, with_codes ? c->b2.wcode.p : (uint32_t*)nullptr, (const uint32_t*)nullptr, true, bi2_tail());
            else
            hipLaunchKernelGGL((bi2_count_kernel<(int)kBi2Sub>), dim3(kBi2Waves), dim3(kWave), 0, c->stream, recsB, b.region, (const uint32_t*)boffB, bs, c->state.p, pl.thr, io.sp_rep, io.sp_cnt,
                               c->b2.wlist.p, c->b2.wcnt.p, b.wcap, want_list, with_codes ? c->b2.wcode.p : (uint32_t*)nullptr, (const uint32_t*)nullptr, true, bi2_tail());
        }
        {
            Prof p(c, COLIBRI_K_PRUNE);
            hipLaunchKernelGGL(bi2_kept_finish_kernel, dim3(kBins + 1), dim3(kBi2BBins), 0, c->stream, c->state.p, bs, pl.thr, pl.res_cap, slice == 0 ? c->b2.headsurv.p : (uint32_t*)nullptr, 4u);
            if (chain) {
                int rcf;
                if ((rcf = chain_compact_fork(c, io, bs, pl))) return rcf;
            } else {
                hipLaunchKernelGGL(bi2_compact_kernel, dim3(1025), dim3(kBlock), 0, c->stream, io.sp_rep, io.sp_cnt, c->state.p, bs, c->res_rep.p, c->res_cnt.p, pl.res_cap);
            }
        }
    }
    if (!want_list) return COLIBRI_OK;
    if (!chain) HIP_TRY(c, hipMemsetAsync(c->b2.bitmap.p + npos / 32, 0, sizeof(uint32_t) * 16, c->stream));
    {
        Prof p(c, COLIBRI_K_LISTS2);
        hipLaunchKernelGGL(bi2_pospart_kernel, dim3(512), dim3(kBi2Threads), 0, c->stream, c->b2.wlist.p, c->b2.wcnt.p, kBi2Waves + b.wextra, b.wcap, bs, c->state.p, c->b2.plist.p, b.pl,
                           with_codes ? (const uint32_t*)c->b2.wcode.p : (const uint32_t*)nullptr, with_codes ? c->b2.pcode.p : (uint32_t*)nullptr, 0u, chain || ids_out != nullptr);
        if (chain) {
            hipLaunchKernelGGL(bi2_headids_kernel, dim3(1), dim3(kBlock), 0, c->stream, (const Bi2State*)bs, (const DevState*)c->state.p, c->b2.headid.p);
            const bool pairs2 = c->b2.pairs2_direct;
            hipLaunchKernelGGL(chain_bitmap_kernel, dim3(b.nbuckets), dim3(kBi2BmThreads), ((size_t)1 << b.pshift) / 8, c->stream, npos, (const Bi2State*)bs, (const uint32_t*)c->b2.plist.p, b.pl,
                               c->state.p, c->b2.bitmap.p, (const uint32_t*)c->b2.pcode.p, (const uint32_t*)c->b2.headid.p, pairs2 ? c->b2.wpre.p : (uint32_t*)nullptr,
                               pairs2 ? c->b2.btot.p : (uint32_t*)nullptr);
            if (ids_out != nullptr || pairs2) {
                int rci;
                if ((rci = chain_ids(c, b, bs, ids_out, (const uint32_t*)c->b2.headid.p, pairs2))) return rci;
            }
            return COLIBRI_OK;
        }
        if (ids_out != nullptr) {
            int rci;
            if ((rci = chain_ids(c, b, bs, ids_out, nullptr))) return rci;
            hipLaunchKernelGGL(bi2_headids_kernel, dim3(1), dim3(kBlock), 0, c->stream, bs, c->state.p, c->b2.headid.p);
        }
        hipLaunchKernelGGL(bi2_bitmap_kernel, dim3(b.nbuckets), dim3(kBi2BmThreads), ((size_t)1 << b.pshift) / 8, c->stream, npos, bs, c->b2.plist.p, b.pl, c->state.p, c->b2.bitmap.p);
        hipLaunchKernelGGL(bi2_list3_kernel, dim3(2048), dim3(kBlock), 0, c->stream, c->cls.p, c->uni_surv.p, npos, c->b2.headsurv.p, c->b2.bitmap.p, c->state.p, c->alist[1].p, nlist, ids_out,
                           ids_out != nullptr ? (const uint32_t*)c->b2.headid.p : (const uint32_t*)nullptr);
    }
    return COLIBRI_OK;
}

int chain_order(colibri_ctx* c, const TrainPlan& pl, int n, bool want_next, uint32_t* ids_out = nullptr ) {
    const uint32_t        npos = pl.npos;
    const bool            wide = chain_wide(npos);
    const uint32_t        nsub = wide ? kBi2SubWide : kBi2Sub, pdrop = wide ? 3u : 0u;
    const Bigram2Plan     b    = bigram2_plan(c, npos, nsub);
    Bi2State* const       bs   = (n & 1) ? c->b2.state2.p : c->b2.state3.p;
    const Bi2State* const prev = n == 3 ? c->b2.state.p : (n & 1) ? c->b2.state3.p : c->b2.state2.p;
    auto* const           recsA = reinterpret_cast<unsigned long long*>(c->recs[0].p);
    auto* const           recsB = reinterpret_cast<unsigned long long*>(c->recs[1].p);
    const BinnedIO        io    = binned_planes(c, pl, false);
    int rcj;
    if ((rcj = chain_compact_join(c))) return rcj;
    {
        Prof p(c, COLIBRI_K_EMIT);
        static const uint32_t grid = chain_grid("COLIBRI_CH_GRID", 768u);
        const uint32_t cap = chain_steps_cap(b.pl);
        hipLaunchKernelGGL(chain_begin_kernel, dim3(kChXcds + kChResetBlocks), dim3(kBi2Threads), 0, c->stream, prev, b.pl, b.nbuckets, reinterpret_cast<uint2*>(c->b2.steps.p), cap,
                           c->b2.steps.p + 2 * (size_t)kChXcds * cap, (const DevState*)c->state.p, bs, c->b2.wcnt.p, kBi2Waves + b.wextra + 1);
        hipLaunchKernelGGL(chain_bits_lds(b.pl) ? chain_emit_kernel<true> : chain_emit_kernel<false>, dim3(grid), dim3(kChThreads), 0, c->stream, (const uint32_t*)c->cls.p, npos, (uint32_t)n, b.clsbits, b.posbits - pdrop, prev,
                           (const uint32_t*)c->b2.plist.p, (const uint32_t*)c->b2.pcode.p, b.pl, reinterpret_cast<const uint2*>(c->b2.steps.p), cap,
                           (const uint32_t*)(c->b2.steps.p + 2 * (size_t)kChXcds * cap),
                           (const uint32_t*)c->b2.bitmap.p, recsA, b.region, nsub, bs, c->state.p, (const uint32_t*)c->b2.headid.p, chain_dbg(), 0u, pdrop);
    }
    {
        Prof p(c, COLIBRI_K_LEVELB2);
        hipLaunchKernelGGL(bi2_levelB_kernel<false>, dim3(b.nslots), dim3(kBi2Threads), 0, c->stream, recsA, recsB, b.region, bs, c->b2.boff.p, c->state.p);
        hipLaunchKernelGGL(bi2_binoff_kernel, dim3(kBins), dim3(kBi2BBins), 0, c->stream, bs, c->b2.boff.p, nsub, c->state.p);
    }
    {
        Prof p(c, COLIBRI_K_BINCOUNT);
        HIP_TRY(c, hipEventRecord(c->b2.ev_fork, c->stream));
        HIP_TRY(c, hipStreamWaitEvent(c->b2.aux, c->b2.ev_fork, 0));
        if (wide)
            hipLaunchKernelGGL((bi2_count_big_kernel<(int)kBi2SubWide, false, false, 2048, true>), dim3(kBi2Waves * kWave / kBi2BigThreads), dim3(kBi2BigThreads), 0, c->stream, recsB, b.region,
                               c->b2.boff.p, bs, c->state.p, pl.thr, io.sp_rep, io.sp_cnt, c->b2.wlist.p, c->b2.wcnt.p, b.wcap, want_next, want_next ? c->b2.wcode.p : (uint32_t*)nullptr,
                               (const uint32_t*)nullptr, kBi2Waves, b.wextra);
        else
            hipLaunchKernelGGL((bi2_count_big_kernel<(int)kBi2Sub>), dim3(kBi2Waves * kWave / kBi2BigThreads), dim3(kBi2BigThreads), 0, c->stream, recsB, b.region, c->b2.boff.p, bs, c->state.p, pl.thr,
                               io.sp_rep, io.sp_cnt, c->b2.wlist.p, c->b2.wcnt.p, b.wcap, want_next, want_next ? c->b2.wcode.p : (uint32_t*)nullptr, (const uint32_t*)nullptr, kBi2Waves, b.wextra);
        if (wide)
            hipLaunchKernelGGL((bi2_count_kernel<(int)kBi2SubWide, false, kBi2WRows, false, 2048, true>), dim3(kBi2Waves), dim3(kWave), 0, c->b2.aux, recsB, b.region, c->b2.boff.p, bs, c->state.p,
                               pl.thr, io.sp_rep, io.sp_cnt, c->b2.wlist.p, c->b2.wcnt.p, b.wcap, want_next, want_next ? c->b2.wcode.p : (uint32_t*)nullptr, (const uint32_t*)nullptr, true, bi2_tail());
        else
            hipLaunchKernelGGL((bi2_count_kernel<(int)kBi2Sub>), dim3(kBi2Waves), dim3(kWave), 0, c->b2.aux, recsB, b.region, c->b2.boff.p, bs, c->state.p, pl.thr, io.sp_rep, io.sp_cnt,
                               c->b2.wlist.p, c->b2.wcnt.p, b.wcap, want_next, want_next ? c->b2.wcode.p : (uint32_t*)nullptr, (const uint32_t*)nullptr, true, bi2_tail());
        HIP_TRY(c, hipEventRecord(c->b2.ev_join, c->b2.aux));
        HIP_TRY(c, hipStreamWaitEvent(c->stream, c->b2.ev_join, 0));
    }
    {
        Prof p(c, COLIBRI_K_PRUNE);
        hipLaunchKernelGGL(bi2_kept_finish_kernel, dim3(kBins + 1), dim3(kBi2BBins), 0, c->stream, c->state.p, bs, pl.thr, pl.res_cap, (uint32_t*)nullptr, 16u);
        int rcf;
        if ((rcf = chain_compact_fork(c, io, bs, pl))) return rcf;
    }
    if (!want_next) return COLIBRI_OK;
    {
        Prof p(c, COLIBRI_K_LISTS2);
        hipLaunchKernelGGL(bi2_pospart_kernel, dim3(512), dim3(kBi2Threads), 0, c->stream, c->b2.wlist.p, c->b2.wcnt.p, kBi2Waves + b.wextra, b.wcap, bs, c->state.p, c->b2.plist.p, b.pl,
                           (const uint32_t*)c->b2.wcode.p, c->b2.pcode.p, 0u, true);
        hipLaunchKernelGGL(chain_bitmap_kernel, dim3(b.nbuckets), dim3(kBi2BmThreads), ((size_t)1 << b.pshift) / 8, c->stream, npos, (const Bi2State*)bs, (const uint32_t*)c->b2.plist.p, b.pl,
                           c->state.p, c->b2.bitmap.p, (const uint32_t*)nullptr, (const uint32_t*)nullptr, c->b2.pairs_direct ? c->b2.wpre.p : (uint32_t*)nullptr,
                           c->b2.pairs_direct ? c->b2.btot.p : (uint32_t*)nullptr);
    }
    if (c->b2.pairs_direct) chain_pairs(c, b, bs, nullptr);
    if (ids_out != nullptr) {
        Prof p(c, COLIBRI_K_RESOLVE);
        int rci;
        if ((rci = chain_ids(c, b, bs, ids_out, nullptr))) return rci;
    }
    return COLIBRI_OK;
}

int skip_pass_chain(colibri_ctx* c, const TrainPlan& pl, int n, uint32_t mask, const uint32_t* left, uint32_t offl, bool l_is_cls, const uint32_t* right, uint32_t offr, bool r_is_cls,
                    uint32_t thr, uint32_t* seglog) {
    const Bigram2Plan b    = bigram2_plan(c, pl.npos);
    Bi2State* const   bs   = (n & 1) ? c->b2.state3.p : c->b2.state2.p;
    auto* const       recsA = reinterpret_cast<unsigned long long*>(c->recs[0].p);
    auto* const       recsB = reinterpret_cast<unsigned long long*>(c->recs[1].p);
    const BinnedIO    io    = binned_planes(c, pl, false);
    Prof              p(c, COLIBRI_K_SKIPGRAM);
    hipLaunchKernelGGL(skip_pass_begin_kernel, dim3(1), dim3(1), 0, c->stream, c->state.p);
    hipLaunchKernelGGL(chain_reset_kernel, dim3(256), dim3(kBlock), 0, c->stream, bs, c->b2.wcnt.p, 0u);
    if (l_is_cls && r_is_cls) {
        hipLaunchKernelGGL(skip_emit_kernel<true>, dim3(kBi2EmitGrid), dim3(kChThreads), 0, c->stream, (const uint32_t*)c->skl, (const uint32_t*)c->skl_n, left, offl, right, offr, 1u, 1u,
                           b.clsbits, b.posbits, recsA, b.region, kBi2Sub, bs, c->state.p, c->b2.head_rows.p);
        hipLaunchKernelGGL(bi2_head_reduce_kernel, dim3(kBi2HeadN / kBlock, kBi2HeadSplit), dim3(kBlock), 0, c->stream, c->b2.head_rows.p, kBi2EmitGrid, bs, c->state.p);
    } else {
        static const uint32_t grid = chain_grid("COLIBRI_CH_GRID", 768u);
        hipLaunchKernelGGL(skip_emit_kernel<false>, dim3(grid), dim3(kChThreads), 0, c->stream, (const uint32_t*)c->skl, (const uint32_t*)c->skl_n, left, offl, right, offr,
                           l_is_cls ? 1u : 0u, r_is_cls ? 1u : 0u, b.clsbits, b.posbits, recsA, b.region, kBi2Sub, bs, c->state.p, (uint32_t*)nullptr);
    }
    hipLaunchKernelGGL(bi2_levelB_kernel<false>, dim3(b.nslots), dim3(kBi2Threads), 0, c->stream, recsA, recsB, b.region, bs, c->b2.boff.p, c->state.p);
    hipLaunchKernelGGL(bi2_binoff_kernel, dim3(kBins), dim3(kBi2BBins), 0, c->stream, bs, c->b2.boff.p, kBi2Sub, c->state.p);
    HIP_TRY(c, hipEventRecord(c->b2.ev_fork, c->stream));
    HIP_TRY(c, hipStreamWaitEvent(c->b2.aux, c->b2.ev_fork, 0));
    hipLaunchKernelGGL((bi2_count_big_kernel<(int)kBi2Sub>), dim3(kBi2Waves * kWave / kBi2BigThreads), dim3(kBi2BigThreads), 0, c->b2.aux, recsB, b.region, c->b2.boff.p, bs, c->state.p, thr,
                       io.sp_rep, io.sp_cnt, c->b2.wlist.p, c->b2.wcnt.p, b.wcap, false, (uint32_t*)nullptr, (const uint32_t*)nullptr, kBi2Waves, b.wextra);
    HIP_TRY(c, hipEventRecord(c->b2.ev_join, c->b2.aux));
    hipLaunchKernelGGL((bi2_count_kernel<(int)kBi2Sub>), dim3(kBi2Waves), dim3(kWave), 0, c->stream, recsB, b.region, c->b2.boff.p, bs, c->state.p, thr, io.sp_rep, io.sp_cnt, c->b2.wlist.p,
                       c->b2.wcnt.p, b.wcap, false, (uint32_t*)nullptr, (const uint32_t*)nullptr, true, bi2_tail());
    HIP_TRY(c, hipStreamWaitEvent(c->stream, c->b2.ev_join, 0));
    hipLaunchKernelGGL(bi2_kept_finish_kernel, dim3(kBins + 1), dim3(kBi2BBins), 0, c->stream, c->state.p, bs, thr, pl.res_cap, (uint32_t*)nullptr, 16u);
    hipLaunchKernelGGL(bi2_compact_kernel, dim3(1025), dim3(kBlock), 0, c->stream, (const uint32_t*)io.sp_rep, (const uint32_t*)io.sp_cnt, (const DevState*)c->state.p, (const Bi2State*)bs,
                       c->res_rep.p, c->res_cnt.p, pl.res_cap, false);
    hipLaunchKernelGGL(skip_pass_end_kernel, dim3(1), dim3(1), 0, c->stream, c->state.p, seglog, (uint32_t)n, mask);
    return COLIBRI_OK;
}

constexpr uint32_t kSplitMaxBits = 3;
bool bigram2_split_fits(const colibri_ctx* c, uint32_t npos) {
    const Bigram2Plan b = bigram2_plan(c, npos);
    return b.sbits >= 1 && b.sbits <= kSplitMaxBits && std::max(2u * b.clsbits, 17u + b.sbits) - 8 + b.posbits <= 64 && !getenv("COLIBRI_RESCAN_SLICES");
}
int bigram2_order_split(colibri_ctx* c, const TrainPlan& pl, bool want_list) {
    const uint32_t    npos = pl.npos, nsurv = c->maxclass / 32 + 1;
    const Bigram2Plan b    = bigram2_plan(c, npos, kBi2SubWide);
    const uint32_t    s    = b.sbits, V = 1u << s;
    auto&             ks   = c->ks;
    int               rc;
    c->b2.keep.drop();
    if ((rc = dev_alloc(c, ks.split, 1)) || (rc = dev_alloc(c, ks.obs, 1)) || (rc = dev_alloc(c, ks.slotbase, kKsSlots)) || (rc = dev_alloc(c, ks.oboff, (size_t)kKsSlots * (kBi2BBins + 1))) ||
        (rc = dev_alloc(c, ks.lcnt, 64)))
        return rc;
    const uint32_t K       = std::max(2u * b.clsbits, 17u + s);
    const uint32_t region  = (uint32_t)(2ull * c->recs[0].n / b.nslots);
    if ((rc = dev_alloc(c, c->b2.wlist, (size_t)npos + ((size_t)V * 2 * kBi2Waves + 64) * kBi2Chunk))) return rc;
    const uint32_t nchunks = (uint32_t)(c->b2.wlist.n / kBi2Chunk);
    if ((rc = dev_alloc(c, c->b2.wcnt, std::max<size_t>(kBi2Waves, nchunks)))) return rc;
    Bi2State* const sbs   = c->b2.state.p;
    Bi2State* const obs   = ks.obs.p;
    auto* const     recsA = reinterpret_cast<unsigned long long*>(c->recs[0].p);
    const bool      direct = !c->split_exact && !getenv("COLIBRI_SPLIT_EXACT");
    auto* const     seg    = reinterpret_cast<unsigned long long*>(c->recs[1].p);
    const uint64_t  extent = std::min<uint64_t>(2ull * c->recs[1].n, 2ull * c->recs[0].n - npos - 2);
    const uint32_t  cap    = (uint32_t)std::min<uint64_t>(extent / ((uint64_t)kKsSlots * kKsWorld), 0xFFFFFFFFull / ((uint64_t)kKsSlots * kKsWorld));
    auto* const     segB   = direct ? reinterpret_cast<unsigned long long*>(c->recs[0].p) + ((size_t)npos + 2) : seg + c->recs[1].n;
    const uint32_t  roomB  = (uint32_t)std::min<uint64_t>(0xFFFFFFFFull, direct ? extent : (uint64_t)c->recs[1].n);
    uint32_t* const nlist = c->alist_n.p + 1;
    uint32_t* const keep  = ks.lcnt.p;
    HIP_TRY(c, hipMemsetAsync(nlist, 0, sizeof(uint32_t), c->stream));
    HIP_TRY(c, hipMemsetAsync(c->b2.wcnt.p, 0, sizeof(uint32_t) * nchunks, c->stream));
    HIP_TRY(c, hipMemsetAsync(keep, 0, sizeof(uint32_t), c->stream));
    HIP_TRY(c, hipMemsetAsync(sbs, 0, sizeof(Bi2State), c->stream));
    HIP_TRY(c, hipMemsetAsync(ks.split.p, 0, sizeof(KsSplitState), c->stream));
    {
        Prof p(c, COLIBRI_K_EMIT2);
        hipLaunchKernelGGL(bi2_emit_kernel, dim3(kBi2EmitGrid), dim3(kBi2Threads), 0, c->stream, c->cls.p, c->uni_surv.p, nsurv, npos, b.clsbits, 0u, 0u, b.posbits, recsA, region, kBi2SubWide, sbs,
                           c->state.p, c->b2.head_rows.p, (uint8_t*)nullptr, K);
        hipLaunchKernelGGL(bi2_head_reduce_kernel, dim3(kBi2HeadN / kBlock, kBi2HeadSplit), dim3(kBlock), 0, c->stream, c->b2.head_rows.p, kBi2EmitGrid, sbs, c->state.p);
    }
    {
        Prof           p(c, COLIBRI_K_SCATTER);
        const KsSplit8 sp{s, b.posbits + K - 8 - s, b.posbits, 0u};
        if (direct) {
            hipLaunchKernelGGL((ks_split_direct_kernel<unsigned long long, KsSplit8, 4>), dim3(kKsSlots), dim3(kKsThreads), 0, c->stream, (const unsigned long long*)recsA, region,
                               (const uint32_t*)sbs->curA, sp, cap, ks.split.p, seg);
        } else {
            hipLaunchKernelGGL((ks_split_hist_kernel<unsigned long long, KsSplit8>), dim3(kKsSlots), dim3(kKsThreads), 0, c->stream, (const unsigned long long*)recsA, region,
                               (const uint32_t*)sbs->curA, sp, ks.split.p);
            hipLaunchKernelGGL(ks_split_scan_kernel, dim3(1), dim3(kKsThreads), 0, c->stream, ks.split.p, s, V, (const DevState*)c->state.p);
            hipLaunchKernelGGL((ks_split_move_kernel<unsigned long long, KsSplit8, 4>), dim3(kKsSlots), dim3(kKsThreads), 0, c->stream, (const unsigned long long*)recsA, region,
                               (const uint32_t*)sbs->curA, sp, (const KsSplitState*)ks.split.p, seg);
            hipLaunchKernelGGL(ks_split_flag_kernel, dim3(1), dim3(1), 0, c->stream, (const KsSplitState*)ks.split.p, (const BinState*)nullptr, c->state.p);
        }
    }
    const BinnedIO io = binned_planes(c, pl, false);
    for (uint32_t v = 0; v < V; ++v) {
        HIP_TRY(c, hipMemsetAsync(obs, 0, sizeof(Bi2State), c->stream));
        if (v == 0)
            HIP_TRY(c, hipMemcpyAsync(obs->headcnt, sbs->headcnt, 2 * sizeof(uint32_t) * kBi2HeadN, hipMemcpyDeviceToDevice, c->stream));
        {
            Prof p(c, COLIBRI_K_LEVELB2);
            hipLaunchKernelGGL(ks_local_init2_kernel, dim3(1), dim3(kKsThreads), 0, c->stream, obs, ks.slotbase.p, (const KsSplitState*)ks.split.p, v, s, K - s, b.posbits + s, (const uint32_t*)keep,
                               roomB, c->state.p);
            hipLaunchKernelGGL(bi2_offsets_kernel, dim3(1), dim3(kBlock), 0, c->stream, obs, 0xFFFFFFFFu, kBi2SubWide, (const DevState*)c->state.p);
            hipLaunchKernelGGL(bi2_levelB_kernel<false>, dim3(kKsSlots), dim3(kBi2Threads), 0, c->stream, (const unsigned long long*)seg, segB, 0xFFFFFFFFu, (const Bi2State*)obs, ks.oboff.p,
                               (const DevState*)c->state.p, (const uint32_t*)ks.slotbase.p);
            hipLaunchKernelGGL(bi2_binoff_kernel, dim3(kBins), dim3(kBi2BBins), 0, c->stream, obs, (const uint32_t*)ks.oboff.p, kBi2SubWide, (const DevState*)c->state.p);
        }
        {
            Prof p(c, COLIBRI_K_COUNT2);
            hipLaunchKernelGGL((bi2_count_big_kernel<(int)kBi2SubWide, true>), dim3(kBi2Waves * kWave / kBi2BigThreads), dim3(kBi2BigThreads), 0, c->stream, (const unsigned long long*)segB, 0u,
                               (const uint32_t*)ks.oboff.p, obs, c->state.p, pl.thr, io.sp_rep, io.sp_cnt, c->b2.wlist.p, c->b2.wcnt.p, nchunks, want_list, (uint32_t*)nullptr,
                               (const uint32_t*)ks.slotbase.p);
            hipLaunchKernelGGL((bi2_count_kernel<(int)kBi2SubWide, true, 16>), dim3(kBi2Waves), dim3(kWave), 0, c->stream, (const unsigned long long*)segB, 0u, (const uint32_t*)ks.oboff.p, obs,
                               c->state.p, pl.thr, io.sp_rep, io.sp_cnt, c->b2.wlist.p, c->b2.wcnt.p, nchunks, want_list, (uint32_t*)nullptr, (const uint32_t*)ks.slotbase.p, true, bi2_tail());
            hipLaunchKernelGGL(ks_keep_chunk_kernel, dim3(1), dim3(1), 0, c->stream, (const Bi2State*)obs, keep);
        }
        {
            Prof p(c, COLIBRI_K_PRUNE);
            hipLaunchKernelGGL(bi2_kept_scan_kernel, dim3(kBins), dim3(kBi2BBins), 0, c->stream, obs, c->state.p);
            hipLaunchKernelGGL(bi2_finish_kernel, dim3(1), dim3(kBlock), 0, c->stream, c->state.p, obs, pl.thr, pl.res_cap, v == 0 ? c->b2.headsurv.p : (uint32_t*)nullptr);
            hipLaunchKernelGGL(bi2_compact_kernel, dim3(1025), dim3(kBlock), 0, c->stream, io.sp_rep, io.sp_cnt, c->state.p, obs, c->res_rep.p, c->res_cnt.p, pl.res_cap);
        }
    }
    if (!want_list) return COLIBRI_OK;
    HIP_TRY(c, hipMemsetAsync(c->b2.bitmap.p + npos / 32, 0, sizeof(uint32_t) * 16, c->stream));
    {
        Prof p(c, COLIBRI_K_LISTS2);
        hipLaunchKernelGGL(bi2_pospart_kernel, dim3(512), dim3(kBi2Threads), 0, c->stream, c->b2.wlist.p, c->b2.wcnt.p, nchunks, kBi2Chunk, sbs, c->state.p, c->b2.plist.p, b.pl,
                           (const uint32_t*)nullptr, (uint32_t*)nullptr, 0u);
        hipLaunchKernelGGL(bi2_bitmap_kernel, dim3(b.nbuckets), dim3(kBi2BmThreads), ((size_t)1 << b.pshift) / 8, c->stream, npos, sbs, c->b2.plist.p, b.pl, c->state.p, c->b2.bitmap.p);
        hipLaunchKernelGGL(bi2_list3_kernel, dim3(2048), dim3(kBlock), 0, c->stream, c->cls.p, c->uni_surv.p, npos, c->b2.headsurv.p, c->b2.bitmap.p, c->state.p, c->alist[1].p, nlist,
                           (uint32_t*)nullptr, (const uint32_t*)nullptr);
    }
    return COLIBRI_OK;
}

template <class KeyFn>
int binned_order(colibri_ctx* c, const TrainPlan& pl, const KeyFn& fn, uint32_t* ids_out, int n, bool use_list, bool need_ids, bool flag_mode = false, bool prefill_ids = false,
                 uint32_t sbits = 0) {
    int rc;
    const BinnedIO io = binned_planes(c, pl, false);
    for (uint32_t slice = 0; slice < (1u << sbits); ++slice) {
        if ((rc = binned_count_stage(c, pl, fn, n, use_list, pl.thr, false, need_ids, flag_mode, false, sbits, slice))) return rc;
        Prof p(c, COLIBRI_K_PRUNE);
        hipLaunchKernelGGL(bin_kept_scan_kernel, dim3(kBins), dim3(kBlock), 0, c->stream, c->state.p, c->binstate.p, pl.res_cap, sbits != 0);
        hipLaunchKernelGGL(compact_bins_kernel, dim3(1024), dim3(kBlock), 0, c->stream, io.sp_rep, io.sp_cnt, c->state.p, c->binstate.p, c->res_rep.p, c->res_cnt.p, pl.res_cap,
                           use_list ? (const uint32_t*)c->alist[n & 1].p : (const uint32_t*)nullptr);
        hipLaunchKernelGGL(bin_advance_prepare_kernel, dim3(1), dim3(1), 0, c->stream, c->state.p, c->binstate.p, sbits != 0);
    }
    if (!need_ids) return COLIBRI_OK;
    if (flag_mode) {
        uint32_t* nlist_out = c->alist_n.p + ((n + 1) & 1);
        HIP_TRY(c, hipMemsetAsync(nlist_out, 0, sizeof(uint32_t), c->stream));
        Prof p(c, COLIBRI_K_RESOLVE);
        hipLaunchKernelGGL(bin_resolve_flags_kernel, dim3(pl.pos_grid), dim3(kBlock), 0, c->stream, c->rep_of.p, c->flags_at.p, c->flag2.p, c->state.p, pl.npos, c->alist[(n + 1) & 1].p,
                           nlist_out);
        return COLIBRI_OK;
    }
    return binned_resolve_stage(c, pl, ids_out, n, use_list, n >= 2, nullptr, 0u, prefill_ids);
}

template <class KeyFn>
int binned_order_split(colibri_ctx* c, const TrainPlan& pl, const KeyFn& fn, uint32_t* ids_out, int n, bool need_ids, bool prefill_ids, uint32_t s) {
    auto& ks = c->ks;
    int   rc;
    if ((rc = dev_alloc(c, ks.split, 1))) return rc;
    const uint32_t  V      = 1u << s;
    const uint32_t  tiles  = blocks_for(pl.npos, kScatTile) + 1 + kASlots;
    const uint32_t  region = (uint32_t)(c->recs[0].n / kASlots);
    const uint32_t* list_in  = c->alist[n & 1].p;
    const uint32_t* nlist_in = c->alist_n.p + (n & 1);
    uint32_t* const ids_at   = need_ids ? c->ids_at.p : nullptr;
    const BinnedIO  io       = binned_planes(c, pl, false);
    Rec* const      seg      = c->recs[1].p;
    Rec* const      R2       = c->recs[0].p + (pl.npos / 2 + 1);
    const bool      direct   = !c->split_exact && !getenv("COLIBRI_SPLIT_EXACT");
    const uint32_t  cap      = (uint32_t)std::min<uint64_t>(c->recs[1].n / ((uint64_t)kKsSlots * kKsWorld), 0xFFFFFFFFull / ((uint64_t)kKsSlots * kKsWorld));
    const uint32_t  room2    = (uint32_t)std::min<uint64_t>(0xFFFFFFFFull, c->recs[0].n - (pl.npos / 2 + 1));
    HIP_TRY(c, hipMemsetAsync(c->binstate.p, 0, sizeof(BinState), c->stream));
    HIP_TRY(c, hipMemsetAsync(ks.split.p, 0, sizeof(KsSplitState), c->stream));
    {
        Prof p(c, COLIBRI_K_EMIT);
        hipLaunchKernelGGL((bin_emit_kernel<KeyFn, true>), dim3(pl.cnt_grid), dim3(kBlock), 0, c->stream, fn, c->recs[0].p, region, c->rep_of.p, c->state.p, c->binstate.p, pl.npos, list_in, nlist_in,
                           ids_at, (uint8_t*)nullptr, 0u, 0u);
    }
    {
        Prof            p(c, COLIBRI_K_SCATTER);
        const KsSplit16 sp{s, 0u};
        const uint4*    recs4 = reinterpret_cast<const uint4*>(c->recs[0].p);
        if (direct) {
            hipLaunchKernelGGL((ks_split_direct_kernel<uint4, KsSplit16, 2>), dim3(kKsSlots), dim3(kKsThreads), 0, c->stream, recs4, region, (const uint32_t*)c->binstate.p->curA, sp, cap, ks.split.p,
                               reinterpret_cast<uint4*>(seg));
        } else {
            hipLaunchKernelGGL((ks_split_hist_kernel<uint4, KsSplit16>), dim3(kKsSlots), dim3(kKsThreads), 0, c->stream, recs4, region, (const uint32_t*)c->binstate.p->curA, sp, ks.split.p);
            hipLaunchKernelGGL(ks_split_scan_kernel, dim3(1), dim3(kKsThreads), 0, c->stream, ks.split.p, s, V, (const DevState*)c->state.p);
            hipLaunchKernelGGL((ks_split_move_kernel<uint4, KsSplit16, 2>), dim3(kKsSlots), dim3(kKsThreads), 0, c->stream, recs4, region, (const uint32_t*)c->binstate.p->curA, sp,
                               (const KsSplitState*)ks.split.p, reinterpret_cast<uint4*>(seg));
            hipLaunchKernelGGL(ks_split_flag_kernel, dim3(1), dim3(1), 0, c->stream, (const KsSplitState*)ks.split.p, (const BinState*)c->binstate.p, c->state.p);
        }
    }
    for (uint32_t v = 0; v < V; ++v) {
        HIP_TRY(c, hipMemsetAsync(c->binstate.p, 0, sizeof(BinState), c->stream));
        {
            Prof p(c, COLIBRI_K_SCATTER);
            hipLaunchKernelGGL(ks_local_init_kernel, dim3(1), dim3(kBlock), 0, c->stream, c->binstate.p, (const KsSplitState*)ks.split.p, v, s, room2, c->state.p);
            hipLaunchKernelGGL(bin_hist2_kernel, dim3(tiles + kBins), dim3(kBlock), 0, c->stream, (const Rec*)seg, (const DevState*)c->state.p, c->binstate.p);
            hipLaunchKernelGGL(bin_scan2_kernel, dim3(kBins), dim3(kBlock), 0, c->stream, c->binstate.p);
            hipLaunchKernelGGL(bin_scatter_kernel, dim3(tiles + kBins), dim3(kBlock), 0, c->stream, (const Rec*)seg, R2, (const DevState*)c->state.p, c->binstate.p);
        }
        {
            Prof p(c, COLIBRI_K_BINCOUNT);
            hipLaunchKernelGGL(bin_count_kernel, dim3(256 * 12), dim3(kBlock), 0, c->stream, (const Rec*)R2, c->state.p, c->binstate.p, pl.thr, io.sp_rep, io.sp_cnt, io.sp_key, ids_at,
                               (uint8_t*)nullptr, false);
        }
        Prof p(c, COLIBRI_K_PRUNE);
        hipLaunchKernelGGL(bin_kept_scan_kernel, dim3(kBins), dim3(kBlock), 0, c->stream, c->state.p, c->binstate.p, pl.res_cap, true);
        hipLaunchKernelGGL(compact_bins_kernel, dim3(1024), dim3(kBlock), 0, c->stream, io.sp_rep, io.sp_cnt, c->state.p, c->binstate.p, c->res_rep.p, c->res_cnt.p, pl.res_cap,
                           (const uint32_t*)c->alist[n & 1].p);
        hipLaunchKernelGGL(bin_advance_prepare_kernel, dim3(1), dim3(1), 0, c->stream, c->state.p, c->binstate.p, true);
    }
    if (!need_ids) return COLIBRI_OK;
    return binned_resolve_stage(c, pl, ids_out, n, true, true, nullptr, 0u, prefill_ids);
}
inline bool binned_split_fits(uint32_t sbits) { return sbits >= 1 && sbits <= kSplitMaxBits && !getenv("COLIBRI_RESCAN_SLICES"); }

int build_skip_list(colibri_ctx* c, const TrainPlan& pl, const uint32_t* gate) {
    const uint32_t ntiles = std::max<uint32_t>(1, blocks_for(pl.npos, kPairTile));
    int            rc;
    if ((rc = dev_alloc(c, c->sklist, (size_t)pl.npos + 1)) || (rc = dev_alloc(c, c->sklist_n, 1)) || (rc = dev_alloc(c, c->idx_cnt, (size_t)ntiles + 2))) return rc;
    Prof p(c, COLIBRI_K_SKIPGRAM);
    hipLaunchKernelGGL(emit_count_kernel, dim3(ntiles), dim3(kPairThreads), 0, c->stream, gate, pl.npos, c->idx_cnt.p, (const DevState*)nullptr);
    hipLaunchKernelGGL(scan_tiles_kernel, dim3(1), dim3(kPairThreads), 0, c->stream, c->idx_cnt.p, ntiles, c->idx_cnt.p + ntiles);
    hipLaunchKernelGGL(list_write_kernel, dim3(ntiles), dim3(kPairThreads), 0, c->stream, gate, pl.npos, (const uint32_t*)c->idx_cnt.p, c->sklist.p, c->sklist_n.p);
    c->skl   = c->sklist.p;
    c->skl_n = c->sklist_n.p;
    return COLIBRI_OK;
}

inline const uint32_t* built_ids(colibri_ctx* c, int n) {
    if (n >= 0 && (size_t)n < c->ids_built.size() && c->ids_built[(size_t)n]) return c->ids[(size_t)n].p;
    (void)fail(c, COLIBRI_ERR_STATE, "internal: the survivor ids of order %d were not built in this run (colibri_train: want_ids)", n);
    return nullptr;
}
inline const uint32_t* part_ids(const colibri_ctx* c, int len) { return (len == 1 && c->ids1_is_cls) ? (const uint32_t*)c->cls.p : (const uint32_t*)c->ids[(size_t)len].p; }

int skipgram_pass(colibri_ctx* c, const TrainPlan& pl, int n, uint32_t mask, const uint32_t* gate, const uint32_t* gate2, uint32_t participants, uint32_t thr, bool count_sources,
                  uint32_t minsrc, uint32_t* found_out, uint32_t* kept_out, int* final_scratch) {
    const std::vector<std::pair<int, int>> parts = mask_parts(mask, n);
    const uint32_t cap = (uint32_t)std::min<uint64_t>(pl.table_slots, (uint64_t)participants + (participants >> 1) + 1024u);
    const uint32_t* left = part_ids(c, parts[0].second);
    uint32_t        offl = (uint32_t)parts[0].first;
    uint32_t*       out  = nullptr;
    int             rc;
    for (size_t j = 1; j < parts.size(); ++j) {
        const bool last = j + 1 == parts.size();
        c->hstate.cap   = cap;
        c->hstate.found = c->hstate.kept = 0;
        if ((rc = write_state(c))) return rc;
        launch_clear(c, pl);
        out = c->scratch[j & 1].p;
        HIP_TRY(c, hipMemsetAsync(out, 0xFF, sizeof(uint32_t) * (size_t)pl.npos, c->stream));
        KeyPair fn{gate, gate2, left, offl, part_ids(c, parts[j].second), (uint32_t)parts[j].first};
        launch_count(c, pl, fn, out, last ? 2 : 0, COLIBRI_K_SKIPGRAM, c->skl, c->skl_n);
        left = out;
        offl = 0;
    }
    const uint32_t* nsrc = nullptr;
    if (count_sources) {
        HIP_TRY(c, hipMemsetAsync(c->nsrc.p, 0, sizeof(uint32_t) * cap, c->stream));
        Prof p(c, COLIBRI_K_SKIPGRAM);
        hipLaunchKernelGGL(skip_sources_kernel, dim3(pl.pos_grid), dim3(kBlock), 0, c->stream, gate, c->res_rep.p, out, c->nsrc.p, c->state.p, pl.npos);
        nsrc = c->nsrc.p;
    }
    launch_prune(c, pl, thr, nsrc, minsrc);
// ... 713 lines not shown
```

### colibri-core_amd/csrc/kshard_api.inc

```

}

namespace {

constexpr uint32_t kKsRouteLen = 32768;
constexpr uint32_t kKsFlatCap  = 16384;

uint32_t ks_range_shift(uint64_t maxclass) {
    uint32_t shift = 12;
    while (shift <= 14 && (maxclass >> shift) >= (uint64_t)kUniBins) ++shift;
    return shift > 14 ? 0u : shift;
}
inline uint32_t ks_log2(int world) {
    uint32_t w = 0;
    while ((1 << w) < world) ++w;
    return w;
}
TrainPlan ks_plan(const colibri_ctx* c) {
    TrainPlan pl{};
    pl.npos     = c->npos;
    pl.thr      = (uint32_t)c->opt.mintokens;
    pl.res_cap  = 0;
    constexpr uint32_t kCountLdsBytes    = kCountTile * 16u + kCountLSlot * 4u + 64u;
    constexpr uint32_t kCountBlocksPerCU = (160u * 1024u / kCountLdsBytes) < 8u ? (160u * 1024u / kCountLdsBytes) : 8u;
// ... 100 lines not shown
    const uint32_t K = std::max(2u * ks.clsbits, 17u + ks.w);
    if (K - 8 + ks.posbits > 64 || K > 48u + ks.w) return fail(c, COLIBRI_ERR_UNSUPPORTED, "key-sharded counting: key and position do not fit a record");
    ks.kbits = K;
    if ((rc = dev_alloc(c, c->cnt1, (size_t)ks.nclasses + 2)) || (rc = dev_alloc(c, c->unistate, 1)) || (rc = dev_alloc(c, c->uni_tail, uni_tail_words(npos))) ||
        (rc = dev_alloc(c, c->uni_rows, (size_t)kUniHeadGrid * kUniHead)) || (rc = dev_alloc(c, c->uni_surv, (size_t)ks.nclasses / 32 + 4 + kBi2SurvLds)))
        return rc;
    if (c->ids.size() < 2) c->ids.resize(2);
    if ((rc = dev_alloc(c, c->ids[0], (size_t)npos + 1)) || (rc = dev_alloc(c, c->ids[1], (size_t)npos + 1))) return rc;
    if ((rc = dev_alloc(c, c->recs[0], ((size_t)npos + (npos >> 2)) / kBins * kBins + (size_t)kBins * kScatTile * 4)) ||
        (rc = dev_alloc(c, c->recs[1], std::max<size_t>((size_t)npos + 1, (size_t)kBins * kScatTile * 4))))
        return rc;
    if ((rc = dev_alloc(c, c->rep_of, (size_t)npos + 1)) || (rc = dev_alloc(c, c->ids_at, (size_t)npos + 1)) || (rc = dev_alloc(c, c->binstate, 1))) return rc;
    if ((rc = dev_alloc(c, c->alist[0], (size_t)npos + 1)) || (rc = dev_alloc(c, c->alist[1], (size_t)npos + 1)) || (rc = dev_alloc(c, c->alist_n, 2))) return rc;
    if ((rc = bigram2_alloc(c, npos, true))) return rc;
    if ((rc = dev_alloc(c, c->state, 1))) return rc;
    if ((rc = dev_alloc(c, ks.split, 1)) || (rc = dev_alloc(c, ks.rstate, 2)) || (rc = dev_alloc(c, ks.stats, 1)) || (rc = dev_alloc(c, ks.ostate, 1)) ||
        (rc = dev_alloc(c, ks.obs, 1)) || (rc = dev_alloc(c, ks.obin, 1)) || (rc = dev_alloc(c, ks.slotbase, kKsSlots)) || (rc = dev_alloc(c, ks.tab_recv, (size_t)kKsWorld * kKs2Bins)) ||
        (rc = dev_alloc(c, ks.headg, 2 * (size_t)kBi2HeadN)) || (rc = dev_alloc(c, ks.oboff, (size_t)kKsSlots * (kBi2BBins + 1))) || (rc = dev_alloc(c, ks.ks2, 1)) ||
        (rc = dev_alloc(c, ks.fbinfo, 1)) || (rc = dev_alloc(c, ks.tab, (size_t)kKsWorld * kKs2Bins)) || (rc = dev_alloc(c, ks.key4, (size_t)npos + 64)) ||
        (rc = dev_alloc(c, ks.posbuf, (size_t)npos + 64)) || (rc = dev_alloc(c, ks.rowtot, kKsSlots)) || (rc = dev_alloc(c, ks.zero8k, 2 * (size_t)kBi2HeadN)) ||
        (rc = dev_alloc(c, ks.small, 16)) || (rc = dev_alloc(c, ks.cbhist, (size_t)kKsSlots * 8 * kBi2BBins)))
        return rc;
    HIP_TRY(c, hipMemsetAsync(ks.zero8k.p, 0, sizeof(uint32_t) * 2 * kBi2HeadN, c->stream));
    ks.indexed = o.indexed != 0;
    ks.gid_off = 0;
    if (ks.indexed && ((rc = pairs_begin(c, npos)) || (rc = dev_alloc(c, ks.fin_gid, (size_t)ks.nclasses + (size_t)npos / 4 + 1024)))) return rc;
    if ((rc = dev_alloc(c, ks.fin_rep, (size_t)ks.nclasses + (size_t)npos / 4 + 1024)) || (rc = dev_alloc(c, ks.fin_cnt, ks.fin_rep.n))) return rc;
    HIP_TRY(c, hipMemsetAsync(ks.stats.p, 0, sizeof(KsStats), c->stream));
    HIP_TRY(c, hipMemsetAsync(ks.ostate.p, 0, sizeof(DevState), c->stream));
    HIP_TRY(c, hipMemsetAsync(c->state.p, 0, sizeof(DevState), c->stream));
    std::memset(&c->hstate, 0, sizeof c->hstate);
    std::memset(&c->stats, 0, sizeof c->stats);
    ks.fin_total   = 0;
    ks.n           = 0;
    ks.pending_uni = false;
    ks.syncs       = 0;
    ks.active      = true;
    return COLIBRI_OK;
}

int colibri_kshard_uni_count(colibri_ctx* c, void** cnt_dev, uint32_t* nclasses) {
    if (!c || !cnt_dev || !nclasses) return COLIBRI_ERR_ARG;
    if (!c->ks.active) return fail(c, COLIBRI_ERR_STATE, "colibri_kshard_begin first");
    HIP_TRY(c, hipSetDevice(c->device));
    int rc;
    if ((rc = uni_count_partitioned(c, c->ks.uni_shift, c->cnt1.p, c->ks.nclasses))) return rc;
    *cnt_dev  = c->cnt1.p;
    *nclasses = c->ks.nclasses;
    c->ks.n   = 1;
    return COLIBRI_OK;
}
int colibri_kshard_uni_apply(colibri_ctx* c) {
    if (!c) return COLIBRI_ERR_ARG;
    auto& ks = c->ks;
    if (!ks.active || ks.n != 1) return fail(c, COLIBRI_ERR_STATE, "colibri_kshard_uni_apply out of order");
    HIP_TRY(c, hipSetDevice(c->device));
    int rc;
    if ((rc = ks_bytes(c, ks.ores_rep, (uint64_t)ks.nclasses + 64)) || (rc = ks_bytes(c, ks.ores_cnt, (uint64_t)ks.nclasses + 64))) return rc;
    const uint32_t wthr = c->opt.mintokens_unigrams > c->opt.mintokens ? (uint32_t)c->opt.mintokens_unigrams : 0u;
    {
        Prof p(c, COLIBRI_K_PRUNE);
        uint32_t* const rep = ks.rank == 0 ? ks.fin_rep.p : ks.ores_rep.p;
        uint32_t* const cnt = ks.rank == 0 ? ks.fin_cnt.p : ks.ores_cnt.p;
        hipLaunchKernelGGL(uni_finish_kernel, dim3(stream_grid(ks.nclasses)), dim3(kBlock), 0, c->stream, (const uint32_t*)c->cnt1.p, (const uint32_t*)nullptr, ks.nclasses,
                           (uint32_t)c->opt.mintokens, ks.ostate.p, rep, cnt, (uint32_t)std::min<size_t>(ks.rank == 0 ? ks.fin_rep.n : ks.ores_rep.n, 0x7FFFFFF0u),
                           reinterpret_cast<uint16_t*>(c->uni_surv.p), false, (uint32_t*)nullptr, wthr);
        if (ks.indexed && ks.rank == 0)
            hipLaunchKernelGGL(ks2_export_gids_kernel, dim3(stream_grid(ks.nclasses)), dim3(kBlock), 0, c->stream, (const uint32_t*)ks.fin_rep.p,
                               (uint32_t)std::min<size_t>(ks.nclasses, ks.fin_gid.n), (const uint32_t*)nullptr, true, ks.fin_gid.p);
        hipLaunchKernelGGL(ks_order_end_kernel, dim3(1), dim3(1), 0, c->stream, ks.ostate.p, c->state.p, ks.stats.p, 1, 0xFFFFFFFFu);
    }
    if (ks.indexed) {
        const TrainPlan pl = ks_plan(c);
        int             rc2;
        hipLaunchKernelGGL(ks2_uni_ids_kernel, dim3(pl.pos_grid), dim3(kBlock), 0, c->stream, (const uint32_t*)c->cls.p, (const uint32_t*)c->cnt1.p, (uint32_t)c->opt.mintokens, c->npos,
                           c->ids[0].p);
        c->hstate.done = 0;
        if ((rc2 = emit_pairs(c, pl, c->ids[0].p, true))) return rc2;
        ++ks.syncs;
        ks.gid_off = ks.nclasses;
    }
    ks.pending_uni = true;
    return COLIBRI_OK;
}

}
namespace {
int ks_settle_uni(colibri_ctx* c) {
    auto& ks = c->ks;
    if (!ks.pending_uni) return COLIBRI_OK;
    uint32_t kept = 0;
    HIP_TRY(c, hipMemcpyAsync(&kept, &ks.stats.p->kept[1], sizeof kept, hipMemcpyDeviceToHost, c->stream));
    HIP_TRY(c, hipStreamSynchronize(c->stream));
    ks.pending_uni = false;
    if (ks.rank == 0) {
        if (kept) c->segments.push_back({0u, kept, 1, kMaskFromClass});
        ks.fin_total = kept;
    }
    return COLIBRI_OK;
}
}
extern "C" {

static uint32_t ks2_bshift(uint64_t est, int world, uint32_t K, uint32_t w) {
    const uint64_t tot = est / (uint64_t)world + 1;
    uint32_t       nb  = 8;
    while (nb < (uint32_t)kBi2BBins && (uint64_t)nb * kBins * 700u < tot) nb <<= 1;
    uint32_t sh = 0;
    while ((uint32_t)kBi2BBins >> sh > nb) ++sh;
    const uint32_t maxsh = K >= 48u + w ? 0u : 48u + w - K;
    return std::min(sh, maxsh);
}

int colibri_kshard_emit(colibri_ctx* c, int n, uint64_t est_records, uint64_t ids_global, int more, void** send_dev, void** tab_dev, uint32_t* tab_words, uint64_t* per_owner,
                        uint32_t* recbytes, void** head_dev, uint64_t* admitted) {
    if (!c || !send_dev || !tab_dev || !tab_words || !per_owner || !recbytes || !head_dev || !admitted || n < 2 || n >= COLIBRI_MAX_ORDER) return COLIBRI_ERR_ARG;
    auto& ks = c->ks;
    if (!ks.active || n != ks.n + 1) return fail(c, COLIBRI_ERR_STATE, "colibri_kshard_emit out of order");
    HIP_TRY(c, hipSetDevice(c->device));
    const uint32_t    npos = c->npos;
    const Bigram2Plan b    = bigram2_plan(c, npos, kBi2SubWide);
    int               rc;
    ks.n = n;
    uint32_t K = ks.kbits, pdrop = 0;
    if (n >= 3) {
        uint32_t idbits = 1;
        while (idbits < 40 && (1ull << idbits) < ids_global + 1) ++idbits;
        K = std::max(idbits + ks.clsbits, 17u + ks.w);
        if (K - 8 + ks.posbits > 64) pdrop = 3;
        if (K - 8 + ks.posbits - pdrop > 64 || K > 48u + ks.w || (pdrop && b.pshift + 3 > ks.posbits))
            return fail(c, COLIBRI_ERR_OVERFLOW, "key-sharded pass of order %d: %u key bits and %u position bits do not fit a record", n, K, ks.posbits);
    }
    const uint32_t bsh = ks2_bshift(est_records, ks.world, K, ks.w);
    Bi2State* const       bs   = n == 2 ? c->b2.state.p : (n & 1) ? c->b2.state2.p : c->b2.state3.p;
    const Bi2State* const prev = n == 3 ? c->b2.state.p : (n & 1) ? c->b2.state3.p : c->b2.state2.p;
    auto* const           recsA = reinterpret_cast<unsigned long long*>(c->recs[0].p);
    auto* const           recsB = reinterpret_cast<unsigned long long*>(c->recs[1].p);
    ks.src_state = bs;
    HIP_TRY(c, hipMemsetAsync(bs, 0, sizeof(Bi2State), c->stream));
    HIP_TRY(c, hipMemsetAsync(ks.ks2.p, 0, sizeof(Ks2State), c->stream));
    hipLaunchKernelGGL(ks2_set_kernel, dim3(1), dim3(1), 0, c->stream, bs, ks.w, bsh);
    if (n == 2) {
        Prof p(c, COLIBRI_K_EMIT2);
        hipLaunchKernelGGL(bi2_emit_kernel, dim3(kBi2EmitGrid), dim3(kBi2Threads), 0, c->stream, c->cls.p, c->uni_surv.p, ks.nclasses / 32 + 1, npos, ks.clsbits, 0u, 0u, ks.posbits, recsA, b.region,
                           kBi2SubWide, bs, c->state.p, c->b2.head_rows.p, (uint8_t*)nullptr, ks.kbits, (more || ks.indexed) ? c->b2.plist.p : (uint32_t*)nullptr,
                           (more || ks.indexed) ? c->b2.pcode.p : (uint32_t*)nullptr, b.pl);
        hipLaunchKernelGGL(bi2_head_reduce_kernel, dim3(kBi2HeadN / kBlock, kBi2HeadSplit), dim3(kBlock), 0, c->stream, c->b2.head_rows.p, kBi2EmitGrid, bs, c->state.p);
        hipLaunchKernelGGL(ks_head_pack_kernel, dim3(kBi2HeadN / kBlock), dim3(kBlock), 0, c->stream, (const Bi2State*)bs, (uint32_t)ks.rank, ks.headg.p);
        *head_dev = ks.headg.p;
    } else {
        Prof           p(c, COLIBRI_K_EMIT);
        const uint32_t cap = chain_steps_cap(b.pl);
        hipLaunchKernelGGL(chain_steps_kernel, dim3(kChXcds), dim3(kBi2Threads), 0, c->stream, prev, b.pl, b.nbuckets, reinterpret_cast<uint2*>(c->b2.steps.p), cap,
                           c->b2.steps.p + 2 * (size_t)kChXcds * cap, (const DevState*)c->state.p);
        hipLaunchKernelGGL(chain_bits_lds(b.pl) ? chain_emit_kernel<true> : chain_emit_kernel<false>, dim3(768), dim3(kChThreads), 0, c->stream, (const uint32_t*)c->cls.p, npos, (uint32_t)n, ks.clsbits, ks.posbits - pdrop, prev,
                           (const uint32_t*)c->b2.plist.p, (const uint32_t*)c->b2.pcode.p, b.pl, reinterpret_cast<const uint2*>(c->b2.steps.p), cap,
                           (const uint32_t*)(c->b2.steps.p + 2 * (size_t)kChXcds * cap), (const uint32_t*)c->b2.bitmap.p, recsA, b.region, kBi2SubWide, bs, c->state.p,
                           (const uint32_t*)c->b2.headid.p, 0u, K, pdrop);
        *head_dev = nullptr;
    }
    {
        Prof p(c, COLIBRI_K_LEVELB2);
        hipLaunchKernelGGL(bi2_levelB_kernel<true>, dim3(b.nslots), dim3(kBi2Threads), 0, c->stream, (const unsigned long long*)recsA, recsB, b.region, (const Bi2State*)bs, c->b2.boff.p,
                           (const DevState*)c->state.p, (const uint32_t*)nullptr, ks.cbhist.p);
    }
    {
        Prof p(c, COLIBRI_K_SCATTER);
        hipLaunchKernelGGL(ks2_hist_kernel, dim3(kBins), dim3(kKsThreads), 0, c->stream, (const uint32_t*)ks.cbhist.p, b.region, (const Bi2State*)bs, ks.w, kBi2SubWide, ks.tab.p, ks.ks2.p);
        hipLaunchKernelGGL(ks2_rows_kernel, dim3(1), dim3(kKsThreads), 0, c->stream, ks.ks2.p, (uint32_t)ks.world, (const DevState*)c->state.p, ks.small.p);
        if ((rc = ks_peek_begin(c)) || (rc = ks_peek(c, 0, ks.ks2.p->dbase, (kKsWorld + 2) * sizeof(uint32_t))) || (rc = ks_peek(c, 12, &c->state.p->radix_overflow, sizeof(uint32_t))) ||
            (rc = ks_peek(c, 13, &bs->overflow, sizeof(uint32_t))) || (rc = ks_peek(c, 14, ks.small.p, sizeof(uint32_t))))
            return rc;
        static const bool move_per_abin = getenv("COLIBRI_KS2_MOVE_ABIN") != nullptr;
        if (move_per_abin)
            hipLaunchKernelGGL(ks2_move_kernel, dim3(kBins), dim3(kKsThreads), 0, c->stream, (const unsigned long long*)recsB, b.region, (const Bi2State*)bs, ks.w, kBi2SubWide,
                               (const uint32_t*)ks.tab.p, (const Ks2State*)ks.ks2.p, (const uint32_t*)c->b2.boff.p, b.pshift, pdrop, ks.key4.p, ks.posbuf.p);
        else
            hipLaunchKernelGGL(ks2_move_slot_kernel, dim3(kBins * kBi2SubWide), dim3(kKsThreads), 0, c->stream, (const unsigned long long*)recsB, b.region, (const Bi2State*)bs, ks.w,
                               kBi2SubWide, (const uint32_t*)ks.tab.p, (const Ks2State*)ks.ks2.p, (const uint32_t*)ks.cbhist.p, b.pshift, pdrop, ks.key4.p, ks.posbuf.p);
    }
    if ((rc = ks_peek_end(c))) return rc;
    const uint32_t* const h = ks.pinned;
    if (ks.pending_uni) {
        uint32_t kept1 = 0;
        HIP_TRY(c, hipMemcpyAsync(&kept1, &ks.stats.p->kept[1], sizeof kept1, hipMemcpyDeviceToHost, ks.side));
        HIP_TRY(c, hipStreamSynchronize(ks.side));
        ks.pending_uni = false;
        if (ks.rank == 0) {
            if (kept1) c->segments.push_back({0u, kept1, 1, kMaskFromClass});
            ks.fin_total = kept1;
        }
    }
    if (h[kKsWorld + 1] || h[12] || h[13])
        return fail(c, COLIBRI_ERR_OVERFLOW, "key-sharded pass of order %d: a record region of the emit kernel or a position list overflowed (%u / %u / %u)", n, h[kKsWorld + 1], h[12], h[13]);
    for (int d = 0; d <= kKsWorld; ++d) ks.sbase[d] = h[std::min(d, ks.world)];
    for (int d = 0; d < ks.world; ++d) per_owner[d] = h[d + 1] - h[d];
    ks.bshift  = bsh;
    *admitted  = h[14];
    *send_dev  = ks.key4.p;
    *tab_dev   = ks.tab.p;
    *tab_words = kKs2Bins;
    *recbytes  = 4;
    return COLIBRI_OK;
}

int colibri_kshard_recv_buffers(colibri_ctx* c, uint64_t nrecords, void** recv_dev, void** tab_recv_dev) {
    if (!c || !recv_dev || !tab_recv_dev) return COLIBRI_ERR_ARG;
    auto& ks = c->ks;
    if (!ks.active || ks.n < 2) return fail(c, COLIBRI_ERR_STATE, "colibri_kshard_recv_buffers out of order");
    if (nrecords >= 0x7FFFFF00ull) return fail(c, COLIBRI_ERR_OVERFLOW, "too many records for one owner");
    HIP_TRY(c, hipSetDevice(c->device));
    int rc;
    if ((rc = ks_bytes(c, ks.rbuf[0], (nrecords + 64) * 4))) return rc;
    *recv_dev     = ks.rbuf[0].p;
    *tab_recv_dev = ks.tab_recv.p;
    return COLIBRI_OK;
}

int colibri_kshard_count(colibri_ctx* c, int n, const uint64_t* per_src, int more, void** fb_dev, uint64_t* fb_per_dst, uint32_t* fb_bytes, void** ex_dev, uint64_t* ex_per_dst,
                         uint64_t* kept_bins) {
    if (!c || !per_src || !fb_dev || !fb_per_dst || !fb_bytes || !ex_dev || !ex_per_dst || !kept_bins) return COLIBRI_ERR_ARG;
    auto& ks = c->ks;
    if (!ks.active || n != ks.n || n < 2) return fail(c, COLIBRI_ERR_STATE, "colibri_kshard_count out of order");
    HIP_TRY(c, hipSetDevice(c->device));
    KsBases  kb{};
    Ks2Segs  sg{};
    uint64_t tot = 0;
    uint32_t ntiles = 0;
    for (int s = 0; s <= kKsWorld; ++s) {
        if (s < kKsWorld) kb.rbase[s] = (uint32_t)tot;
        sg.base[s]  = (uint32_t)tot;
        sg.tbase[s] = ntiles;
        if (s < ks.world) {
            tot += per_src[s];
            ntiles += blocks_for(per_src[s], kKs2Tile);
        }
    }
    if (tot >= 0x7FFFFF00ull) return fail(c, COLIBRI_ERR_OVERFLOW, "too many records for one owner");
    const uint32_t nrec = (uint32_t)tot, thr = (uint32_t)c->opt.mintokens;
    const uint32_t rescap = nrec + 2 * (uint32_t)kBi2HeadN;
    int            rc;
    if ((rc = ks_bytes(c, ks.osp_rep, (uint64_t)nrec + 64)) || (rc = ks_bytes(c, ks.osp_cnt, (uint64_t)nrec + 64)) || (rc = ks_bytes(c, ks.ores_rep, rescap)) ||
        (rc = ks_bytes(c, ks.ores_cnt, rescap)) || (rc = ks_bytes(c, ks.exs, (uint64_t)rescap * 8)) || (rc = ks_bytes(c, ks.code_at, (uint64_t)nrec + 64)) ||
        (rc = ks_bytes(c, ks.tcnt, (uint64_t)ntiles + 8)) || (rc = ks_bytes(c, ks.fbs, ((uint64_t)nrec + nrec / 32 + 64) * 4)))
        return rc;
    const uint32_t nl_ex = blocks_for(rescap, kKsRouteLen);
    if ((rc = ks_bytes(c, ks.lcnt, 2 * ((uint64_t)nl_ex * kKsWorld + 64))) || (rc = ks_bytes(c, ks.loff, 2 * ((uint64_t)nl_ex * kKsWorld + 64)))) return rc;
    DevState* const ost = ks.ostate.p;
    Bi2State* const obs = ks.obs.p;
    auto* const     R   = reinterpret_cast<const unsigned long long*>(ks.rbuf[0].p);
    if (ks.indexed) more = 1;
    const uint32_t* const headg = n == 2 ? (const uint32_t*)ks.headg.p : (const uint32_t*)ks.zero8k.p;
    HIP_TRY(c, hipMemsetAsync(obs, 0, sizeof(Bi2State), c->stream));
    {
        Prof p(c, COLIBRI_K_LEVELB2);
        hipLaunchKernelGGL(ks2_owner_rows_kernel, dim3(kBins), dim3(kBi2BBins), 0, c->stream, (const uint32_t*)ks.tab_recv.p, (uint32_t)ks.world, ks.oboff.p, ks.rowtot.p);
        hipLaunchKernelGGL(ks2_owner_init_kernel, dim3(1), dim3(kKsThreads), 0, c->stream, obs, ks.slotbase.p, (const uint32_t*)ks.rowtot.p, kb, ks.bshift);
        hipLaunchKernelGGL(bi2_offsets_kernel, dim3(1), dim3(kBlock), 0, c->stream, obs, 0xFFFFFFFFu, (uint32_t)kKsWorld, (const DevState*)ost);
        hipLaunchKernelGGL(bi2_binoff_kernel, dim3(kBins), dim3(kBi2BBins), 0, c->stream, obs, (const uint32_t*)ks.oboff.p, (uint32_t)kKsWorld, (const DevState*)ost);
    }
    {
        Prof p(c, COLIBRI_K_COUNT2);
        HIP_TRY(c, hipEventRecord(c->b2.ev_fork, c->stream));
        HIP_TRY(c, hipStreamWaitEvent(c->b2.aux, c->b2.ev_fork, 0));
        hipLaunchKernelGGL((bi2_count_big_kernel<(int)kKsWorld, true, true>), dim3(kBi2Waves * kWave / kBi2BigThreads), dim3(kBi2BigThreads), 0, c->b2.aux, R, 0u, (const uint32_t*)ks.oboff.p, obs, ost,
                           thr, ks.osp_rep.p, ks.osp_cnt.p, ks.code_at.p, (uint32_t*)nullptr, 0u, more != 0, (uint32_t*)nullptr, (const uint32_t*)ks.slotbase.p);
        HIP_TRY(c, hipEventRecord(c->b2.ev_join, c->b2.aux));
        hipLaunchKernelGGL((bi2_count_kernel<(int)kKsWorld, true, 16, true>), dim3(kBi2Waves), dim3(kWave), 0, c->stream, R, 0u, (const uint32_t*)ks.oboff.p, obs, ost, thr, ks.osp_rep.p,
                           ks.osp_cnt.p, ks.code_at.p, (uint32_t*)nullptr, 0u, more != 0, (uint32_t*)nullptr, (const uint32_t*)ks.slotbase.p, true, bi2_tail());
        HIP_TRY(c, hipStreamWaitEvent(c->stream, c->b2.ev_join, 0));
    }
    {
        Prof p(c, COLIBRI_K_PRUNE);
        hipLaunchKernelGGL(bi2_kept_scan_kernel, dim3(kBins), dim3(kBi2BBins), 0, c->stream, obs, (const DevState*)ost);
        hipLaunchKernelGGL(ks_finish2_kernel, dim3(1), dim3(kBlock), 0, c->stream, ost, obs, headg, (uint32_t)ks.rank, thr, rescap, c->b2.headsurv.p);
        hipLaunchKernelGGL(ks2_compact_kernel, dim3(1025), dim3(kBlock), 0, c->stream, (const uint32_t*)ks.osp_rep.p, (const uint32_t*)ks.osp_cnt.p, (const Bi2State*)obs,
                           (const Bi2State*)c->b2.state.p, headg, kb, (uint32_t)ks.world, ks.ores_rep.p, ks.ores_cnt.p, rescap);
        const Ks2RouteExports exsp{ks.ores_rep.p, ks.ores_cnt.p, &ost->kept, kKsRouteLen, (uint32_t)ks.rank};
        ks_route_count(c, exsp, nl_ex, (uint32_t)ks.world, ks.rstate.p + 1, 1);
        if (more && ntiles) {
            hipLaunchKernelGGL(ks2_fb_count_kernel, dim3(std::min<uint32_t>(blocks_for(ntiles, kKsThreads / kWave), 2048u)), dim3(kKsThreads), 0, c->stream, (const uint32_t*)ks.code_at.p, sg, ntiles, ks.tcnt.p);
            hipLaunchKernelGGL(scan_tiles_kernel, dim3(1), dim3(kPairThreads), 0, c->stream, ks.tcnt.p, ntiles, ks.tcnt.p + ntiles);
        } else {
            HIP_TRY(c, hipMemsetAsync(ks.tcnt.p, 0, sizeof(uint32_t) * ((size_t)ntiles + 1), c->stream));
        }
        hipLaunchKernelGGL(ks2_fb_info_kernel, dim3(1), dim3(1), 0, c->stream, (const uint32_t*)ks.tcnt.p, sg, (uint32_t)(more ? ks.world : 0), ntiles, (const Bi2State*)obs, ks.fbinfo.p);
        if ((rc = ks_peek_begin(c)) || (rc = ks_peek(c, 0, ks.rstate.p + 1, sizeof(KsRouteState))) || (rc = ks_peek(c, 32, ost, 16 * sizeof(uint32_t))) ||
            (rc = ks_peek(c, 64, ks.fbinfo.p, sizeof(Ks2FbInfo))))
            return rc;
        ks_route_move<Ks2RouteExports, 4>(c, exsp, nl_ex, (uint32_t)ks.world, reinterpret_cast<unsigned long long*>(ks.exs.p), 1);
        if (more && ntiles)
            hipLaunchKernelGGL(ks2_fb_write_kernel, dim3(std::min<uint32_t>(blocks_for(ntiles, kKsThreads / kWave), 2048u)), dim3(kKsThreads), 0, c->stream, (const uint32_t*)ks.code_at.p, sg, ntiles, (const uint32_t*)ks.tcnt.p,
                               (const Ks2FbInfo*)ks.fbinfo.p, (const Bi2State*)obs, reinterpret_cast<uint32_t*>(ks.fbs.p));
    }
    hipLaunchKernelGGL(ks_order_end_kernel, dim3(1), dim3(1), 0, c->stream, ost, c->state.p, ks.stats.p, n, 0xFFFFFFFFu);
    if ((rc = ks_peek_end(c))) return rc;
    KsRouteState hr{};
    DevState     hs{};
    Ks2FbInfo    fi{};
    std::memcpy(&hr, ks.pinned, sizeof hr);
    std::memcpy(&hs, ks.pinned + 32, 16 * sizeof(uint32_t));
    std::memcpy(&fi, ks.pinned + 64, sizeof fi);
    if (hs.overflow || hs.radix_overflow)
        return fail(c, COLIBRI_ERR_OVERFLOW, "key-sharded pass of order %d: %s", n,
                    hs.overflow ? "owner result buffer exhausted" : hs.radix_overflow == 5 ? "a record slot overflowed" : "a final bin outgrew its LDS table");
    for (int d = 0; d < ks.world; ++d) {
        fb_per_dst[d] = more ? fi.off[d + 1] - fi.off[d] : 0;
// ... 184 lines not shown
```

Baseline: 199,400 M patterns counted/s.

## Merge chain step lists per bucket, batch compaction copies, fuse head-id assignment

Adds a merged step-numbering mode. Each bucket's shard lists are concatenated into one logical sequence, so emit and id kernels walk fewer, fuller steps, and the emit loop prefetches one step further ahead. Head-id assignment moves into the kept-finish kernel, which removes a separate single-block launch. An optional ballot-batched compaction path copies several small bins per wave round. These trade extra index arithmetic per load and more code paths against fewer partially filled steps and fewer launches.

```diff
diff --git a/colibri-core_amd/csrc/bigram2.hpp b/colibri-core_amd/csrc/bigram2.hpp
--- a/colibri-core_amd/csrc/bigram2.hpp
+++ b/colibri-core_amd/csrc/bigram2.hpp
@@ -1408,7 +1408,7 @@
     }
 }
 __global__ __launch_bounds__(kBi2BBins) void bi2_kept_finish_kernel(DevState* __restrict__ st, Bi2State* __restrict__ bs, uint32_t threshold, uint32_t res_cap,
-                                                                     uint32_t* __restrict__ headsurv_keep, uint32_t ovf_code) {
+                                                                     uint32_t* __restrict__ headsurv_keep, uint32_t ovf_code, uint32_t* __restrict__ headid_out) {
     if (st->done) return;
     __shared__ uint32_t inL[kBi2BBins], outL[kBi2BBins], wsumL[8], beforeL;
     if (blockIdx.x < (uint32_t)kBins) {
@@ -1426,8 +1426,9 @@
         return;
     }
     static_assert(kBi2HeadN == kBlock * 16 && kBins == kBlock && kBi2BBins >= kBlock, "16 head keys per lane of the first 256");
-    const bool low = threadIdx.x < (uint32_t)kBlock;
-    uint32_t   htot, ftot, hftot, tot;
+    const bool     low = threadIdx.x < (uint32_t)kBlock;
+    const uint32_t rb  = st->res_total + st->kept;
+    uint32_t       htot, ftot, hftot, tot;
     bi2_block_scan<kBi2BBins>(low ? bs->found_part[threadIdx.x] : 0u, &ftot, wsumL);
     bi2_block_scan<kBi2BBins>(low ? bs->kept_part[threadIdx.x] : 0u, &tot, wsumL);
     uint32_t hk = 0, hf = 0, bits = 0;
@@ -1446,11 +1447,16 @@
     }
     const uint32_t ho = bi2_block_scan<kBi2BBins>(hk, &htot, wsumL);
     if (low) bs->headbase[threadIdx.x] = ho;
+    if (low && headid_out != nullptr) {
+        uint32_t r = rb + tot + ho;
+#pragma unroll
+        for (int q = 0; q < 16; ++q) headid_out[threadIdx.x * 16 + q] = (bits & (1u << q)) ? r++ : kInvalid;
+    }
     bi2_block_scan<kBi2BBins>(hf, &hftot, wsumL);
     if (threadIdx.x == 0) {
         bs->kept_head = htot;
         bs->ran       = 1;
-        bs->res_base  = st->res_total + st->kept;
+        bs->res_base  = rb;
         st->found += ftot + hftot;
         st->kept += tot + htot;
         if ((uint64_t)bs->res_base + tot + htot > res_cap) st->overflow = 1;
@@ -1461,12 +1467,63 @@
         st->id_base = (uint32_t)next;
     }
 }
+constexpr int kBi2CompactBatch = 4;
 __global__ __launch_bounds__(kBlock) void bi2_compact_kernel(const uint32_t* __restrict__ sp_rep, const uint32_t* __restrict__ sp_cnt, const DevState* __restrict__ st,
                                                               const Bi2State* __restrict__ bs, uint32_t* __restrict__ res_rep, uint32_t* __restrict__ res_cnt, uint32_t res_cap,
-                                                              bool beside = false ) {
+                                                              bool beside = false ,
+                                                              bool serial = true) {
     if (beside ? !bs->ran : st->done != 0) return;
     const uint32_t res_base = bs->res_base, lane = threadIdx.x & (kWave - 1);
-    if (blockIdx.x + 1 < gridDim.x) {
+    if (blockIdx.x + 1 < gridDim.x && !serial) {
+        static_assert(kBi2Final % kWave == 0 && kWave == 64, "64 bins per wave and round, a 64-bit ballot");
+        const uint32_t nwaves = (gridDim.x - 1) * (kBlock / kWave), kept_bins = bs->kept_bins;
+        for (uint32_t grp = blockIdx.x * (kBlock / kWave) + threadIdx.x / kWave; grp < (uint32_t)kBi2Final / kWave; grp += nwaves) {
+            const uint32_t g   = grp * kWave + lane;
+            const uint32_t f   = ((g & (uint32_t)(kBins - 1)) * kBi2BBins) + (g >> 8);
+            const uint32_t off = bs->binkept[f];
+            const uint32_t end = (f + 1 < (uint32_t)kBi2Final) ? bs->binkept[f + 1] : kept_bins;
+            const uint32_t src = bs->binoff[f];
+            const uint32_t n   = end - off;
+            unsigned long long todo = __ballot(n != 0);
+            while (todo) {
+                uint32_t o[kBi2CompactBatch], m[kBi2CompactBatch], s[kBi2CompactBatch], vr[kBi2CompactBatch], vc[kBi2CompactBatch];
+#pragma unroll
+                for (int k = 0; k < kBi2CompactBatch; ++k) {
+                    m[k] = 0u;
+                    o[k] = s[k] = 0u;
+                    if (todo) {
+                        const int b = __builtin_ctzll(todo);
+                        todo &= todo - 1ull;
+                        o[k] = (uint32_t)__builtin_amdgcn_readlane((int)off, b);
+                        m[k] = (uint32_t)__builtin_amdgcn_readlane((int)n, b);
+                        s[k] = (uint32_t)__builtin_amdgcn_readlane((int)src, b);
+                    }
+                }
+#pragma unroll
+                for (int k = 0; k < kBi2CompactBatch; ++k) {
+                    vr[k] = lane < m[k] ? sp_rep[s[k] + lane] : 0u;
+                    vc[k] = lane < m[k] ? sp_cnt[s[k] + lane] : 0u;
+                }
+#pragma unroll
+                for (int k = 0; k < kBi2CompactBatch; ++k) {
+                    const uint32_t r = res_base + o[k] + lane;
+                    if (lane < m[k] && r < res_cap) {
+                        res_rep[r] = vr[k];
+                        res_cnt[r] = vc[k];
+                    }
+                }
+#pragma unroll
+                for (int k = 0; k < kBi2CompactBatch; ++k)
+                    for (uint32_t j = lane + kWave; j < m[k]; j += kWave) {
+                        const uint32_t r = res_base + o[k] + j;
+                        if (r < res_cap) {
+                            res_rep[r] = sp_rep[s[k] + j];
+                            res_cnt[r] = sp_cnt[s[k] + j];
+                        }
+                    }
+            }
+        }
+    } else if (blockIdx.x + 1 < gridDim.x) {
         const uint32_t nwaves = (gridDim.x - 1) * (kBlock / kWave);
         for (uint32_t g = blockIdx.x * (kBlock / kWave) + threadIdx.x / kWave; g < (uint32_t)kBi2Final; g += nwaves) {
             const uint32_t f   = ((g & (uint32_t)(kBins - 1)) * kBi2BBins) + (g >> 8);
diff --git a/colibri-core_amd/csrc/chain.hpp b/colibri-core_amd/csrc/chain.hpp
--- a/colibri-core_amd/csrc/chain.hpp
+++ b/colibri-core_amd/csrc/chain.hpp
@@ -308,25 +308,74 @@
             if (base < cap) table[(size_t)x * cap + base] = make_uint2(first[q] + k * (uint32_t)kChStep, chain_step_pack(min((uint32_t)kChStep, n[q] - k * (uint32_t)kChStep), bucket[q]));
     if (threadIdx.x == 0) nsteps[x] = min(total, cap);
 }
+static_assert(kChCatLists == kChLists, "chain_step.hpp's sequence has a part per list of a bucket");
+__device__ __forceinline__ ChainCat chain_cat_of(const Bi2State* __restrict__ prev, const Bi2Lists& pl, uint32_t bucket, bool merge) {
+    uint32_t len[kChLists], first[kChLists];
+#pragma unroll
+    for (uint32_t l = 0; l < kChLists; ++l) len[l] = prev->pcur[bi2_pc(l * kBi2Buckets + bucket)];
+#pragma unroll
+    for (uint32_t l = 0; l < kChLists; ++l) {
+        uint32_t f, lcap;
+        bi2_list_of(pl, l, bucket, f, lcap);
+        len[l]   = merge ? min((uint32_t)__builtin_amdgcn_readfirstlane((int)len[l]), lcap) : (l == 0 ? 0xFFFFFFFFu : 0u);
+        first[l] = merge ? f : 0u;
+    }
+    return chain_cat_make(len, first);
+}
+__device__ __forceinline__ bool chain_number_steps_merged(const Bi2State* __restrict__ prev, const Bi2Lists& pl, uint32_t nbuckets, uint2* __restrict__ table, uint32_t cap,
+                                                          uint32_t* __restrict__ nsteps, uint32_t x, uint32_t* wsumL, uint32_t merge_max) {
+    constexpr uint32_t kLanes = kBi2Threads / (kBi2Buckets / kChXcds);
+    static_assert(kLanes * (kBi2Buckets / kChXcds) == kBi2Threads && kLanes >= 1, "whole groups of lanes per bucket");
+    const uint32_t bkt = x + kChXcds * (threadIdx.x / kLanes), j = threadIdx.x % kLanes;
+    uint32_t       total = 0;
+    if (bkt < nbuckets) {
+#pragma unroll
+        for (uint32_t l = 0; l < kChLists; ++l) {
+            uint32_t first, lcap;
+            bi2_list_of(pl, l, bkt, first, lcap);
+            total += min(prev->pcur[bi2_pc(l * kBi2Buckets + bkt)], lcap);
+        }
+    }
+    const uint32_t ns = chain_cat_steps(total, (uint32_t)kChStep);
+    uint32_t       all;
+    const uint32_t excl = bi2_block_scan<kBi2Threads>(j == 0 ? ns : 0u, &all, wsumL);
+    if (all > merge_max) return false;
+    const uint32_t base = j == 0 ? excl : excl - ns;
+    for (uint32_t k = j; k < ns; k += kLanes)
+        if (base + k < cap) table[(size_t)x * cap + base + k] = make_uint2(chain_cat_entry_x(k, (uint32_t)kChStep), chain_cat_entry_y(k, total, (uint32_t)kChStep, bkt));
+    if (threadIdx.x == 0) nsteps[x] = min(all, cap);
+    return true;
+}
+__device__ __forceinline__ void chain_number_steps_auto(const Bi2State* __restrict__ prev, const Bi2Lists& pl, uint32_t nbuckets, uint2* __restrict__ table, uint32_t cap,
+                                                        uint32_t* __restrict__ nsteps, uint32_t x, uint32_t* wsumL, uint32_t merge_max) {
+    const bool merged = merge_max != 0u && chain_number_steps_merged(prev, pl, nbuckets, table, cap, nsteps, x, wsumL, merge_max);
+    if (!merged) chain_number_steps(prev, pl, nbuckets, table, cap, nsteps, x, wsumL);
+    if (threadIdx.x == 0) nsteps[kChXcds + x] = merged ? 1u : 0u;
+}
 __global__ __launch_bounds__(kBi2Threads) void chain_steps_kernel(const Bi2State* __restrict__ prev, Bi2Lists pl, uint32_t nbuckets, uint2* __restrict__ table, uint32_t cap,
-                                                                   uint32_t* __restrict__ nsteps, const DevState* __restrict__ st) {
+                                                                   uint32_t* __restrict__ nsteps, const DevState* __restrict__ st, uint32_t merge_max) {
     if (st->done) return;
     __shared__ uint32_t wsumL[kBi2Threads / kWave];
-    chain_number_steps(prev, pl, nbuckets, table, cap, nsteps, blockIdx.x, wsumL);
+    chain_number_steps_auto(prev, pl, nbuckets, table, cap, nsteps, blockIdx.x, wsumL, merge_max);
 }
 constexpr uint32_t kChResetBlocks = 64;
 __global__ __launch_bounds__(kBi2Threads) void chain_begin_kernel(const Bi2State* __restrict__ prev, Bi2Lists pl, uint32_t nbuckets, uint2* __restrict__ table, uint32_t cap,
                                                                    uint32_t* __restrict__ nsteps, const DevState* __restrict__ st, Bi2State* __restrict__ bs, uint32_t* __restrict__ wcnt,
-                                                                   uint32_t nwcnt) {
+                                                                   uint32_t nwcnt, uint32_t merge_max) {
     if (blockIdx.x >= kChXcds) {
         chain_clear_state(bs, wcnt, nwcnt, (blockIdx.x - kChXcds) * kBi2Threads + threadIdx.x, (gridDim.x - kChXcds) * kBi2Threads);
         return;
     }
     if (st->done) return;
     __shared__ uint32_t wsumL[kBi2Threads / kWave];
-    chain_number_steps(prev, pl, nbuckets, table, cap, nsteps, blockIdx.x, wsumL);
+    chain_number_steps_auto(prev, pl, nbuckets, table, cap, nsteps, blockIdx.x, wsumL, merge_max);
 }
 inline uint32_t chain_steps_cap(const Bi2Lists& pl) { return (kBi2Buckets / kChXcds) * (kBi2Shards * (pl.pcap / kChStep + 1) + ((1u << pl.pshift) / kChStep + 1)); }
+inline uint32_t chain_merge_max(uint32_t grid, uint32_t run) {
+    const char* const e = getenv("COLIBRI_CH_MERGE");
+    return (e && e[0] == '0' && e[1] == 0) ? 0u : (grid / kChXcds) * run;
+}
+inline size_t chain_steps_words(const Bi2Lists& pl) { return 2 * (size_t)kChXcds * chain_steps_cap(pl) + 2 * kChXcds; }
 
 template <bool BITS_LDS>
 __global__ __launch_bounds__(kChThreads, kChEmitBlocks* kChThreads / 256) void chain_emit_kernel(
@@ -345,8 +394,9 @@
     const uint32_t        sub = blockIdx.x % nsub;
     const uint32_t        x = blockIdx.x % kChXcds, nper = gridDim.x / kChXcds, ns = nsteps[x];
     const uint2* const    tab = table + (size_t)x * cap;
+    const bool            merge = nsteps[kChXcds + x] != 0u;
     const uint32_t        rbase = kfix ? 0u : prev->res_base;
-    uint32_t              k = chain_run_first(blockIdx.x / kChXcds, kRun), k1 = chain_run_next(k, nper, kRun);
+    uint32_t              k = chain_run_first(blockIdx.x / kChXcds, kRun), k1 = chain_run_next(k, nper, kRun), ka = chain_run_next(k1, nper, kRun);
     constexpr uint32_t kSlicePer = BITS_LDS ? ((1u << kChSliceShift) / 128u + kChThreads - 1) / kChThreads : 1u;
     const uint32_t     sw = (1u << pl.pshift) / 32u + 1u, tw = (npos + 31u) / 32u + 16u;
     uint32_t           stail = 0, snw = 0;
@@ -375,15 +425,16 @@
         const uint2 e = s < ns ? tab[s] : make_uint2(0u, 0u);
         return make_uint2((uint32_t)__builtin_amdgcn_readfirstlane((int)e.x), (uint32_t)__builtin_amdgcn_readfirstlane((int)e.y));
     };
-    uint2 e1 = entry(k);
-    auto  load_pairs = [&]() {
+    uint2    e1 = entry(k);
+    ChainCat c1 = chain_cat_of(prev, pl, chain_step_bucket(e1.y), merge);
+    auto     load_pairs = [&]() {
         const uint32_t np = chain_step_pairs(e1.y);
 #pragma unroll
         for (int q = 0; q < kChPer; ++q) {
-            const uint32_t j = q * kChThreads + threadIdx.x;
+            const uint32_t j = q * kChThreads + threadIdx.x, i = chain_cat_index(c1, e1.x + j);
             ok[q]            = j < np;
-            ps[q]            = ok[q] ? plist[(size_t)e1.x + j] : 0u;
-            code[q]          = ok[q] ? pcode[(size_t)e1.x + j] : 0u;
+            ps[q]            = ok[q] ? plist[i] : 0u;
+            code[q]          = ok[q] ? pcode[i] : 0u;
         }
     };
     load_pairs();
@@ -393,7 +444,9 @@
         slice_store();
         __syncthreads();
     }
-    e1 = entry(k1);
+    e1       = entry(k1);
+    c1       = chain_cat_of(prev, pl, chain_step_bucket(e1.y), merge);
+    uint2 e2 = entry(ka);
     KP_INIT(4);
     while (k < ns) {
         uint32_t p2[kChPer], c2[kChPer], w[kChPer], cn[kChPer];
@@ -419,8 +472,11 @@
             bcur   = chain_step_bucket(e1.y);
         }
         k  = k1;
-        k1 = chain_run_next(k1, nper, kRun);
-        e1 = entry(k1);
+        k1 = ka;
+        ka = chain_run_next(ka, nper, kRun);
+        e1 = e2;
+        c1 = chain_cat_of(prev, pl, chain_step_bucket(e1.y), merge);
+        e2 = entry(ka);
         uint32_t cnt = 0;
 #pragma unroll
         for (int q = 0; q < kChPer; ++q) {
@@ -542,19 +598,22 @@
 
 __global__ __launch_bounds__(kChThreads) void chain_ids_kernel(const uint32_t* __restrict__ plist, const uint32_t* __restrict__ pcode, const uint2* __restrict__ table, uint32_t cap,
                                                                 const uint32_t* __restrict__ nsteps, const Bi2State* __restrict__ bs, const DevState* __restrict__ st,
-                                                                uint32_t* __restrict__ ids, const uint32_t* __restrict__ headid = nullptr ) {
+                                                                uint32_t* __restrict__ ids, const uint32_t* __restrict__ headid ,
+                                                                Bi2Lists pl ) {
     if (st->done) return;
     const uint32_t     x = blockIdx.x % kChXcds, nper = gridDim.x / kChXcds, ns = nsteps[x], res_base = bs->res_base;
+    const bool         merge = nsteps[kChXcds + x] != 0u;
     const uint2* const tab = table + (size_t)x * cap;
     for (uint32_t k = blockIdx.x / kChXcds; k < ns; k += nper) {
         const uint2    e  = tab[k];
-        const uint32_t np = chain_step_pairs(e.y);
+        const uint32_t np = chain_step_pairs(e.y), ex = (uint32_t)__builtin_amdgcn_readfirstlane((int)e.x);
+        const ChainCat ct = chain_cat_of(bs, pl, (uint32_t)__builtin_amdgcn_readfirstlane((int)chain_step_bucket(e.y)), merge);
         uint32_t       ps[kChPer], cd[kChPer];
 #pragma unroll
         for (int q = 0; q < kChPer; ++q) {
-            const uint32_t j = q * kChThreads + threadIdx.x;
-            ps[q]            = j < np ? plist[(size_t)e.x + j] : kInvalid;
-            cd[q]            = j < np ? pcode[(size_t)e.x + j] : 0u;
+            const uint32_t j = q * kChThreads + threadIdx.x, i = chain_cat_index(ct, ex + j);
+            ps[q]            = j < np ? plist[i] : kInvalid;
+            cd[q]            = j < np ? pcode[i] : 0u;
         }
 #pragma unroll
         for (int q = 0; q < kChPer; ++q)
@@ -669,7 +728,7 @@
                                                                   const uint32_t* __restrict__ bitmap, const uint32_t* __restrict__ wpre, const uint32_t* __restrict__ btot,
                                                                   uint32_t nbuckets, uint32_t pshift, const uint4* __restrict__ blocks, const unsigned long long* __restrict__ chain,
                                                                   int which, uint64_t pcap, unsigned long long* __restrict__ pairs, uint32_t* __restrict__ pay, uint32_t sb, uint32_t tb,
-                                                                  const uint32_t* __restrict__ headid) {
+                                                                  const uint32_t* __restrict__ headid, Bi2Lists pl ) {
     if (st->done) return;
     __shared__ uint32_t bbaseL[kBi2Buckets], wsumL[kChThreads / kWave];
     static_assert(kBi2Buckets == 2 * kChThreads, "two buckets per lane");
@@ -682,19 +741,21 @@
     }
     __syncthreads();
     const uint32_t     x = blockIdx.x % kChXcds, nper = gridDim.x / kChXcds, ns = nsteps[x], res_base = bs->res_base;
+    const bool         merge = nsteps[kChXcds + x] != 0u;
     const uint2* const tab   = table + (size_t)x * cap;
     const uint64_t     obase = chain[which];
     const uint32_t     tmask = tb >= 32 ? 0xFFFFFFFFu : (1u << tb) - 1u;
     for (uint32_t k = blockIdx.x / kChXcds; k < ns; k += nper) {
         const uint2    e  = tab[k];
-        const uint32_t np = chain_step_pairs(e.y);
+        const uint32_t np = chain_step_pairs(e.y), ex = (uint32_t)__builtin_amdgcn_readfirstlane((int)e.x);
+        const ChainCat ct = chain_cat_of(bs, pl, (uint32_t)__builtin_amdgcn_readfirstlane((int)chain_step_bucket(e.y)), merge);
         uint32_t       ps[kChPer], cd[kChPer], bw[kChPer], wp[kChPer];
         uint4          r[kChPer];
 #pragma unroll
         for (int q = 0; q < kChPer; ++q) {
-            const uint32_t j = q * kChThreads + threadIdx.x;
-            ps[q]            = j < np ? plist[(size_t)e.x + j] : kInvalid;
-            cd[q]            = j < np ? pcode[(size_t)e.x + j] : 0u;
+            const uint32_t j = q * kChThreads + threadIdx.x, i = chain_cat_index(ct, ex + j);
+            ps[q]            = j < np ? plist[i] : kInvalid;
+            cd[q]            = j < np ? pcode[i] : 0u;
         }
 #pragma unroll
         for (int q = 0; q < kChPer; ++q) {
diff --git a/colibri-core_amd/csrc/chain_step.hpp b/colibri-core_amd/csrc/chain_step.hpp
--- a/colibri-core_amd/csrc/chain_step.hpp
+++ b/colibri-core_amd/csrc/chain_step.hpp
@@ -14,6 +14,46 @@
 COLIBRI_STEP_HD uint32_t chain_step_pairs(uint32_t y) { return y & ((1u << kChStepPairBits) - 1u); }
 COLIBRI_STEP_HD uint32_t chain_step_bucket(uint32_t y) { return y >> kChStepPairBits; }
 
+constexpr uint32_t kChCatLists = 9;
+struct ChainCat {
+    uint32_t end[kChCatLists], hop[kChCatLists];
+};
+COLIBRI_STEP_HD ChainCat chain_cat_make(const uint32_t (&len)[kChCatLists], const uint32_t (&first)[kChCatLists]) {
+    ChainCat c;
+    uint32_t sum = 0, before = 0;
+#pragma unroll
+    for (uint32_t l = 0; l < kChCatLists; ++l) {
+        const uint32_t delta = first[l] - sum;
+        c.hop[l]             = delta - before;
+        before               = delta;
+        sum += len[l];
+        c.end[l] = sum;
+    }
+    return c;
+}
+COLIBRI_STEP_HD ChainCat chain_cat_single() {
+    ChainCat c;
+#pragma unroll
+    for (uint32_t l = 0; l < kChCatLists; ++l) {
+        c.end[l] = 0xFFFFFFFFu;
+        c.hop[l] = 0u;
+    }
+    return c;
+}
+COLIBRI_STEP_HD uint32_t chain_cat_total(const ChainCat& c) { return c.end[kChCatLists - 1]; }
+COLIBRI_STEP_HD uint32_t chain_cat_index(const ChainCat& c, uint32_t o) {
+    uint32_t i = o + c.hop[0];
+#pragma unroll
+    for (uint32_t l = 1; l < kChCatLists; ++l) i += o >= c.end[l - 1] ? c.hop[l] : 0u;
+    return i;
+}
+COLIBRI_STEP_HD uint32_t chain_cat_steps(uint32_t total, uint32_t step) { return total / step + (total % step != 0u ? 1u : 0u); }
+COLIBRI_STEP_HD uint32_t chain_cat_entry_x(uint32_t k, uint32_t step) { return k * step; }
+COLIBRI_STEP_HD uint32_t chain_cat_entry_y(uint32_t k, uint32_t total, uint32_t step, uint32_t bucket) {
+    const uint32_t left = total - k * step;
+    return chain_step_pack(left < step ? left : step, bucket);
+}
+
 COLIBRI_STEP_HD uint32_t chain_run_first(uint32_t k, uint32_t run) { return k * run; }
 COLIBRI_STEP_HD uint32_t chain_run_next(uint32_t s, uint32_t nper, uint32_t run) { return (s + 1u) % run != 0u ? s + 1u : s + 1u + (nper - 1u) * run; }
 
diff --git a/colibri-core_amd/csrc/colibri_hip.hip b/colibri-core_amd/csrc/colibri_hip.hip
--- a/colibri-core_amd/csrc/colibri_hip.hip
+++ b/colibri-core_amd/csrc/colibri_hip.hip
@@ -1051,7 +1051,7 @@
         HIP_TRY(c, hipEventCreateWithFlags(&c->b2.ev_fork2, hipEventDisableTiming));
         HIP_TRY(c, hipEventCreateWithFlags(&c->b2.ev_join2, hipEventDisableTiming));
     }
-    if (chain && ((rc = dev_alloc(c, c->b2.steps, 2 * (size_t)kChXcds * chain_steps_cap(b.pl) + kChXcds)) || (rc = dev_alloc(c, c->b2.state2, 1)) || (rc = dev_alloc(c, c->b2.state3, 1)) || (rc = dev_alloc(c, c->b2.wcode, (size_t)(kBi2Waves + b.wextra) * b.wcap)) ||
+    if (chain && ((rc = dev_alloc(c, c->b2.steps, chain_steps_words(b.pl))) || (rc = dev_alloc(c, c->b2.state2, 1)) || (rc = dev_alloc(c, c->b2.state3, 1)) || (rc = dev_alloc(c, c->b2.wcode, (size_t)(kBi2Waves + b.wextra) * b.wcap)) ||
                   (rc = dev_alloc(c, c->b2.pcode, b.listn)) || (rc = dev_alloc(c, c->b2.headid, kBi2HeadN))))
         return rc;
     if (b.sbits) {
@@ -1066,11 +1066,20 @@
     }
     return COLIBRI_OK;
 }
-int chain_compact_fork(colibri_ctx* c, const BinnedIO& io, const Bi2State* bs, const TrainPlan& pl) {
+inline bool bi2_compact_serial() {
+    const char* const e = getenv("COLIBRI_BI2_COMPACT");
+    return !(e && e[0] == '1' && e[1] == 0);
+}
+int chain_compact_fork(colibri_ctx* c, const BinnedIO& io, const Bi2State* bs, const TrainPlan& pl, bool last = false) {
+    if (last) {
+        hipLaunchKernelGGL(bi2_compact_kernel, dim3(1025), dim3(kBlock), 0, c->stream, (const uint32_t*)io.sp_rep, (const uint32_t*)io.sp_cnt, (const DevState*)c->state.p, bs, c->res_rep.p,
+                           c->res_cnt.p, pl.res_cap, true, bi2_compact_serial());
+        return COLIBRI_OK;
+    }
     HIP_TRY(c, hipEventRecord(c->b2.ev_fork2, c->stream));
     HIP_TRY(c, hipStreamWaitEvent(c->b2.aux, c->b2.ev_fork2, 0));
     hipLaunchKernelGGL(bi2_compact_kernel, dim3(1025), dim3(kBlock), 0, c->b2.aux, (const uint32_t*)io.sp_rep, (const uint32_t*)io.sp_cnt, (const DevState*)c->state.p, bs, c->res_rep.p,
-                       c->res_cnt.p, pl.res_cap, true);
+                       c->res_cnt.p, pl.res_cap, true, bi2_compact_serial());
     HIP_TRY(c, hipEventRecord(c->b2.ev_join2, c->b2.aux));
     c->b2.compact_pending = true;
     return COLIBRI_OK;
@@ -1137,10 +1146,10 @@
     HIP_TRY(c, hipMemsetAsync(ids, 0xFF, sizeof(uint32_t) * (size_t)c->npos, c->stream));
     const uint32_t cap = chain_steps_cap(b.pl);
     hipLaunchKernelGGL(chain_steps_kernel, dim3(kChXcds), dim3(kBi2Threads), 0, c->stream, bs, b.pl, b.nbuckets, reinterpret_cast<uint2*>(c->b2.steps.p), cap,
-                       c->b2.steps.p + 2 * (size_t)kChXcds * cap, (const DevState*)c->state.p);
+                       c->b2.steps.p + 2 * (size_t)kChXcds * cap, (const DevState*)c->state.p, chain_merge_max(chain_grid("COLIBRI_IDS_GRID", 1024u), 1u));
     static const uint32_t ids_grid = chain_grid("COLIBRI_IDS_GRID", 1024u);
     hipLaunchKernelGGL(chain_ids_kernel, dim3(ids_grid), dim3(kChThreads), 0, c->stream, (const uint32_t*)c->b2.plist.p, (const uint32_t*)c->b2.pcode.p,
-                       reinterpret_cast<const uint2*>(c->b2.steps.p), cap, (const uint32_t*)(c->b2.steps.p + 2 * (size_t)kChXcds * cap), bs, (const DevState*)c->state.p, ids, headid);
+                       reinterpret_cast<const uint2*>(c->b2.steps.p), cap, (const uint32_t*)(c->b2.steps.p + 2 * (size_t)kChXcds * cap), bs, (const DevState*)c->state.p, ids, headid, b.pl);
     return COLIBRI_OK;
 }
 void chain_pairs(colibri_ctx* c, const Bigram2Plan& b, const Bi2State* bs, const uint32_t* headid) {
@@ -1148,13 +1157,13 @@
     const uint32_t cap  = chain_steps_cap(b.pl);
     const uint64_t pcap = c->pairs[0].n;
     hipLaunchKernelGGL(chain_steps_kernel, dim3(kChXcds), dim3(kBi2Threads), 0, c->stream, bs, b.pl, b.nbuckets, reinterpret_cast<uint2*>(c->b2.steps.p), cap,
-                       c->b2.steps.p + 2 * (size_t)kChXcds * cap, (const DevState*)c->state.p);
+                       c->b2.steps.p + 2 * (size_t)kChXcds * cap, (const DevState*)c->state.p, chain_merge_max(chain_grid("COLIBRI_IDS_GRID", 1024u), 1u));
     static const uint32_t grid = chain_grid("COLIBRI_IDS_GRID", 1024u);
     hipLaunchKernelGGL(chain_pairs_kernel, dim3(grid), dim3(kChThreads), 0, c->stream, (const uint32_t*)c->b2.plist.p, (const uint32_t*)c->b2.pcode.p,
                        reinterpret_cast<const uint2*>(c->b2.steps.p), cap, (const uint32_t*)(c->b2.steps.p + 2 * (size_t)kChXcds * cap), bs, (const DevState*)c->state.p,
                        (const uint32_t*)c->b2.bitmap.p, (const uint32_t*)c->b2.wpre.p, (const uint32_t*)c->b2.btot.p, b.nbuckets, b.pshift,
                        reinterpret_cast<const uint4*>(c->pos_blocks.p), (const unsigned long long*)c->pair_chain.p, c->pair_pass, pcap, c->pairs[0].p,
-                       c->pair_split ? reinterpret_cast<uint32_t*>(c->pairs[0].p) + pcap : (uint32_t*)nullptr, c->pair_sb, c->pair_tb, headid);
+                       c->pair_split ? reinterpret_cast<uint32_t*>(c->pairs[0].p) + pcap : (uint32_t*)nullptr, c->pair_sb, c->pair_tb, headid, b.pl);
     hipLaunchKernelGGL(pairs_advance_kernel, dim3(1), dim3(1), 0, c->stream, c->pair_chain.p, c->pair_pass, (const uint32_t*)&c->state.p->valid, pcap);
     c->pair_pass ^= 1;
 }
@@ -1165,7 +1174,7 @@
         int rc;
         if (b.sbits != 0 || !want_list) return fail(c, COLIBRI_ERR_STATE, "bigram2_order: ids need the single-pass form with lists");
         if ((rc = dev_alloc(c, c->b2.wcode, (size_t)(kBi2Waves + b.wextra) * b.wcap)) || (rc = dev_alloc(c, c->b2.pcode, (size_t)kBi2Shards * kBi2Buckets * b.pl.pcap + 64)) ||
-            (rc = dev_alloc(c, c->b2.headid, kBi2HeadN)) || (rc = dev_alloc(c, c->b2.steps, 2 * (size_t)kChXcds * chain_steps_cap(b.pl) + kChXcds)))
+            (rc = dev_alloc(c, c->b2.headid, kBi2HeadN)) || (rc = dev_alloc(c, c->b2.steps, chain_steps_words(b.pl))))
             return rc;
     }
     if (chain && b.sbits != 0) return fail(c, COLIBRI_ERR_STATE, "bigram2_order: the chained orders need the single-pass form");
@@ -1241,12 +1250,13 @@
         }
         {
             Prof p(c, COLIBRI_K_PRUNE);
-            hipLaunchKernelGGL(bi2_kept_finish_kernel, dim3(kBins + 1), dim3(kBi2BBins), 0, c->stream, c->state.p, bs, pl.thr, pl.res_cap, slice == 0 ? c->b2.headsurv.p : (uint32_t*)nullptr, 4u);
+            hipLaunchKernelGGL(bi2_kept_finish_kernel, dim3(kBins + 1), dim3(kBi2BBins), 0, c->stream, c->state.p, bs, pl.thr, pl.res_cap, slice == 0 ? c->b2.headsurv.p : (uint32_t*)nullptr, 4u,
+                               (chain && want_list) ? c->b2.headid.p : (uint32_t*)nullptr);
             if (chain) {
                 int rcf;
-                if ((rcf = chain_compact_fork(c, io, bs, pl))) return rcf;
+                if ((rcf = chain_compact_fork(c, io, bs, pl, !want_list))) return rcf;
             } else {
-                hipLaunchKernelGGL(bi2_compact_kernel, dim3(1025), dim3(kBlock), 0, c->stream, io.sp_rep, io.sp_cnt, c->state.p, bs, c->res_rep.p, c->res_cnt.p, pl.res_cap);
+                hipLaunchKernelGGL(bi2_compact_kernel, dim3(1025), dim3(kBlock), 0, c->stream, io.sp_rep, io.sp_cnt, c->state.p, bs, c->res_rep.p, c->res_cnt.p, pl.res_cap, false, bi2_compact_serial());
             }
         }
     }
@@ -1257,7 +1267,6 @@
         hipLaunchKernelGGL(bi2_pospart_kernel, dim3(512), dim3(kBi2Threads), 0, c->stream, c->b2.wlist.p, c->b2.wcnt.p, kBi2Waves + b.wextra, b.wcap, bs, c->state.p, c->b2.plist.p, b.pl,
                            with_codes ? (const uint32_t*)c->b2.wcode.p : (const uint32_t*)nullptr, with_codes ? c->b2.pcode.p : (uint32_t*)nullptr, 0u, chain || ids_out != nullptr);
         if (chain) {
-            hipLaunchKernelGGL(bi2_headids_kernel, dim3(1), dim3(kBlock), 0, c->stream, (const Bi2State*)bs, (const DevState*)c->state.p, c->b2.headid.p);
             const bool pairs2 = c->b2.pairs2_direct;
             hipLaunchKernelGGL(chain_bitmap_kernel, dim3(b.nbuckets), dim3(kBi2BmThreads), ((size_t)1 << b.pshift) / 8, c->stream, npos, (const Bi2State*)bs, (const uint32_t*)c->b2.plist.p, b.pl,
                                c->state.p, c->b2.bitmap.p, (const uint32_t*)c->b2.pcode.p, (const uint32_t*)c->b2.headid.p, pairs2 ? c->b2.wpre.p : (uint32_t*)nullptr,
@@ -1297,7 +1306,8 @@
         static const uint32_t grid = chain_grid("COLIBRI_CH_GRID", 768u);
         const uint32_t cap = chain_steps_cap(b.pl);
         hipLaunchKernelGGL(chain_begin_kernel, dim3(kChXcds + kChResetBlocks), dim3(kBi2Threads), 0, c->stream, prev, b.pl, b.nbuckets, reinterpret_cast<uint2*>(c->b2.steps.p), cap,
-                           c->b2.steps.p + 2 * (size_t)kChXcds * cap, (const DevState*)c->state.p, bs, c->b2.wcnt.p, kBi2Waves + b.wextra + 1);
+                           c->b2.steps.p + 2 * (size_t)kChXcds * cap, (const DevState*)c->state.p, bs, c->b2.wcnt.p, kBi2Waves + b.wextra + 1,
+                           chain_merge_max(grid, chain_bits_lds(b.pl) ? kChRun : 1u));
         hipLaunchKernelGGL(chain_bits_lds(b.pl) ? chain_emit_kernel<true> : chain_emit_kernel<false>, dim3(grid), dim3(kChThreads), 0, c->stream, (const uint32_t*)c->cls.p, npos, (uint32_t)n, b.clsbits, b.posbits - pdrop, prev,
                            (const uint32_t*)c->b2.plist.p, (const uint32_t*)c->b2.pcode.p, b.pl, reinterpret_cast<const uint2*>(c->b2.steps.p), cap,
                            (const uint32_t*)(c->b2.steps.p + 2 * (size_t)kChXcds * cap),
@@ -1330,9 +1340,9 @@
     }
     {
         Prof p(c, COLIBRI_K_PRUNE);
-        hipLaunchKernelGGL(bi2_kept_finish_kernel, dim3(kBins + 1), dim3(kBi2BBins), 0, c->stream, c->state.p, bs, pl.thr, pl.res_cap, (uint32_t*)nullptr, 16u);
+        hipLaunchKernelGGL(bi2_kept_finish_kernel, dim3(kBins + 1), dim3(kBi2BBins), 0, c->stream, c->state.p, bs, pl.thr, pl.res_cap, (uint32_t*)nullptr, 16u, (uint32_t*)nullptr);
         int rcf;
-        if ((rcf = chain_compact_fork(c, io, bs, pl))) return rcf;
+        if ((rcf = chain_compact_fork(c, io, bs, pl, !want_next))) return rcf;
     }
     if (!want_next) return COLIBRI_OK;
     {
@@ -1381,9 +1391,9 @@
     hipLaunchKernelGGL((bi2_count_kernel<(int)kBi2Sub>), dim3(kBi2Waves), dim3(kWave), 0, c->stream, recsB, b.region, c->b2.boff.p, bs, c->state.p, thr, io.sp_rep, io.sp_cnt, c->b2.wlist.p,
                        c->b2.wcnt.p, b.wcap, false, (uint32_t*)nullptr, (const uint32_t*)nullptr, true, bi2_tail());
     HIP_TRY(c, hipStreamWaitEvent(c->stream, c->b2.ev_join, 0));
-    hipLaunchKernelGGL(bi2_kept_finish_kernel, dim3(kBins + 1), dim3(kBi2BBins), 0, c->stream, c->state.p, bs, thr, pl.res_cap, (uint32_t*)nullptr, 16u);
+    hipLaunchKernelGGL(bi2_kept_finish_kernel, dim3(kBins + 1), dim3(kBi2BBins), 0, c->stream, c->state.p, bs, thr, pl.res_cap, (uint32_t*)nullptr, 16u, (uint32_t*)nullptr);
     hipLaunchKernelGGL(bi2_compact_kernel, dim3(1025), dim3(kBlock), 0, c->stream, (const uint32_t*)io.sp_rep, (const uint32_t*)io.sp_cnt, (const DevState*)c->state.p, (const Bi2State*)bs,
-                       c->res_rep.p, c->res_cnt.p, pl.res_cap, false);
+                       c->res_rep.p, c->res_cnt.p, pl.res_cap, false, bi2_compact_serial());
     hipLaunchKernelGGL(skip_pass_end_kernel, dim3(1), dim3(1), 0, c->stream, c->state.p, seglog, (uint32_t)n, mask);
     return COLIBRI_OK;
 }
@@ -1472,7 +1482,7 @@
             Prof p(c, COLIBRI_K_PRUNE);
             hipLaunchKernelGGL(bi2_kept_scan_kernel, dim3(kBins), dim3(kBi2BBins), 0, c->stream, obs, c->state.p);
             hipLaunchKernelGGL(bi2_finish_kernel, dim3(1), dim3(kBlock), 0, c->stream, c->state.p, obs, pl.thr, pl.res_cap, v == 0 ? c->b2.headsurv.p : (uint32_t*)nullptr);
-            hipLaunchKernelGGL(bi2_compact_kernel, dim3(1025), dim3(kBlock), 0, c->stream, io.sp_rep, io.sp_cnt, c->state.p, obs, c->res_rep.p, c->res_cnt.p, pl.res_cap);
+            hipLaunchKernelGGL(bi2_compact_kernel, dim3(1025), dim3(kBlock), 0, c->stream, io.sp_rep, io.sp_cnt, c->state.p, obs, c->res_rep.p, c->res_cnt.p, pl.res_cap, false, bi2_compact_serial());
         }
     }
     if (!want_list) return COLIBRI_OK;
diff --git a/colibri-core_amd/csrc/kshard_api.inc b/colibri-core_amd/csrc/kshard_api.inc
--- a/colibri-core_amd/csrc/kshard_api.inc
+++ b/colibri-core_amd/csrc/kshard_api.inc
@@ -276,7 +276,7 @@
         Prof           p(c, COLIBRI_K_EMIT);
         const uint32_t cap = chain_steps_cap(b.pl);
         hipLaunchKernelGGL(chain_steps_kernel, dim3(kChXcds), dim3(kBi2Threads), 0, c->stream, prev, b.pl, b.nbuckets, reinterpret_cast<uint2*>(c->b2.steps.p), cap,
-                           c->b2.steps.p + 2 * (size_t)kChXcds * cap, (const DevState*)c->state.p);
+                           c->b2.steps.p + 2 * (size_t)kChXcds * cap, (const DevState*)c->state.p, 0u);
         hipLaunchKernelGGL(chain_bits_lds(b.pl) ? chain_emit_kernel<true> : chain_emit_kernel<false>, dim3(768), dim3(kChThreads), 0, c->stream, (const uint32_t*)c->cls.p, npos, (uint32_t)n, ks.clsbits, ks.posbits - pdrop, prev,
                            (const uint32_t*)c->b2.plist.p, (const uint32_t*)c->b2.pcode.p, b.pl, reinterpret_cast<const uint2*>(c->b2.steps.p), cap,
                            (const uint32_t*)(c->b2.steps.p + 2 * (size_t)kChXcds * cap), (const uint32_t*)c->b2.bitmap.p, recsA, b.region, kBi2SubWide, bs, c->state.p,
```

Result: slower. 193,900 M patterns counted/s (-2.8%).
